# igd-geo/schwarzwald

Hardware: AMD Instinct MI355X
Metric: Mpoints/s end-to-end tile (Morton+sort+sample) (higher is better)
Workload: dtype u64 keys / f64 positions

## Files before the change

schwarzwald_amd/csrc/swz_api.hip:

```cpp
#include <algorithm>
#include <cstring>

#include "swz_device.h"
#include "swz_internal.h"

int swz_ctx::get(const char* name, size_t bytes, void** out) {
  swz::DevBuf& b = bufs[name];
  if (bytes == 0) bytes = 16;
  if (b.cap < bytes) {
    const size_t old_cap = b.cap;
    if (b.ptr) {
      SWZ_HIP(this, hipStreamSynchronize(stream));
      free_buf(b);
    }
    size_t want = bytes + bytes / 16;
    const size_t minimal = (want + 255) & ~size_t(255);
    if (old_cap) {
      if (strncmp(name, "tl_", 3) == 0 || strncmp(name, "tiler_store", 11) == 0) want = std::max(want, 2 * old_cap);
      else want = std::max(want, std::min(2 * old_cap, bytes + (size_t(1) << 30)));
    }
    want = (want + 255) & ~size_t(255);
    hipError_t e = hipMalloc(&b.ptr, want);
    if (const char* fa = opt("SWZ_FAIL_ALLOC")) {
      const size_t fl = strlen(fa);
      const bool hit = fl && fa[fl - 1] == '*' ? strncmp(fa, name, fl - 1) == 0 : strcmp(fa, name) == 0;
      if (e == hipSuccess && hit) {
        (void)hipFree(b.ptr);
        b.ptr = nullptr;
        e = hipErrorOutOfMemory;
      }
    }
    if (e == hipErrorOutOfMemory) {
      (void)hipGetLastError();
      SWZ_HIP(this, hipStreamSynchronize(stream));
      for (auto& kv : bufs) {
        const std::string& nm = kv.first;
        const bool level_scratch = nm.compare(0, 3, "md_") == 0 || nm.compare(0, 3, "sp_") == 0 || nm.compare(0, 3, "pm_") == 0;
        const bool shared_root = md_shard_root_published && nm.size() >= 3 && nm.compare(nm.size() - 3, 3, "_sr") == 0;
        const bool tiler_scratch = tiler_scratch_dead && nm.compare(0, 3, "tl_") == 0;
        if ((level_scratch || tiler_scratch) && !shared_root && kv.second.ptr && kv.second.epoch < scratch_epoch && &kv.second != &b)
          free_buf(kv.second);
      }
      e = hipMalloc(&b.ptr, want);
      if (e == hipErrorOutOfMemory && want > minimal) {
        (void)hipGetLastError();
        want = minimal;
        e = hipMalloc(&b.ptr, want);
      }
    }
    if (e != hipSuccess) {
      b.ptr = nullptr;
      std::vector<std::pair<size_t, std::string>> held;
      size_t total = 0;
      for (const auto& kv : bufs) {
        if (kv.second.host) continue;
        total += kv.second.cap;
        if (kv.second.cap) held.emplace_back(kv.second.cap, kv.first);
      }
      std::sort(held.rbegin(), held.rend());
      size_t free_b = 0, total_b = 0;
      (void)hipMemGetInfo(&free_b, &total_b);
      std::string top;
      for (size_t i = 0; i < held.size() && i < 14; ++i)
        top += " " + held[i].second + "=" + std::to_string(held[i].first >> 20) + "M";
      return fail(SWZ_ERR_HIP, std::string("hipMalloc(") + name + ", " + std::to_string(want) + " bytes): " + hipGetErrorString(e) +
                                 "; workspace holds " + std::to_string(total >> 20) + " MiB, device free " +
                                 std::to_string(free_b >> 20) + " of " + std::to_string(total_b >> 20) + " MiB; largest:" + top);
    }
    b.cap = want;
    if (const char* e = opt("SWZ_POISON")) {
      const char* only = opt("SWZ_POISON_ONLY");
      if (!only || strstr(name, only)) SWZ_HIP(this, hipMemsetAsync(b.ptr, atoi(e), want, stream));
    }
  }
  b.epoch = scratch_epoch;
  *out = b.ptr;
  return SWZ_OK;
}

void swz_ctx::release_all() {
  if (stream) (void)hipStreamSynchronize(stream);
  for (auto& kv : bufs) free_buf(kv.second);
  bufs.clear();
}

void swz_ctx::free_buf(swz::DevBuf& b) {
  if (b.ptr && b.ptr == sbi_clean_ptr) sbi_clean_ptr = nullptr;
  if (b.ptr && b.ptr == mq_qpos_buf) mq_qpos_buf = nullptr;
  if (b.ptr) (void)(b.host ? hipHostFree(b.ptr) : hipFree(b.ptr));
  b.ptr = nullptr;
  b.cap = 0;
  b.host = false;
}

uint64_t swz_ctx::held_bytes() const {
  uint64_t s = 0;
  for (const auto& kv : bufs)
    if (!kv.second.host) s += kv.second.cap;
  return s;
}

uint64_t swz_ctx::held_host_bytes() const {
  uint64_t s = 0;
  for (const auto& kv : bufs)
    if (kv.second.host) s += kv.second.cap;
  return s;
}

hipEvent_t swz_ctx::take_event() {
  if (!event_pool.empty()) {
    hipEvent_t e = event_pool.back();
    event_pool.pop_back();
    return e;
  }
  hipEvent_t e = nullptr;
  (void)hipEventCreate(&e);
  return e;
}

void swz_ctx::prof_begin(const char*) {
  if (!profile) return;
  cur_e0_ = take_event();
  (void)hipEventRecord(cur_e0_, stream);
}

void swz_ctx::prof_end(const char* name, uint64_t launches, uint64_t bytes) {
  if (!profile || !cur_e0_) return;
  hipEvent_t e1 = take_event();
  (void)hipEventRecord(e1, stream);
  pending.push_back({name, cur_e0_, e1, launches, bytes});
  cur_e0_ = nullptr;
}

void swz_ctx::prof_collect() {
  for (auto& p : pending) {
    float ms = 0.f;
    if (hipEventSynchronize(p.e1) == hipSuccess && hipEventElapsedTime(&ms, p.e0, p.e1) == hipSuccess) {
      swz::KernelStat& k = kstats[p.name];
      k.launches += p.launches;
      k.total_ms += ms;
      k.bytes += p.bytes;
    }
    event_pool.push_back(p.e0);
    event_pool.push_back(p.e1);
  }
  pending.clear();
}

int swz::read_u32(swz_ctx* c, const uint32_t* d, uint32_t* h) {
  SWZ_HIP(c, hipMemcpyAsync(h, d, 4, hipMemcpyDeviceToHost, c->stream));
  SWZ_HIP(c, hipStreamSynchronize(c->stream));
  return SWZ_OK;
}

int swz::check_params(swz_ctx* c, const swz_tile_params* p) {
  if (!p) return c->fail(SWZ_ERR_BAD_ARG, "params must not be NULL");
  if (p->sampler < SWZ_RANDOM_GRID || p->sampler > SWZ_MIN_DISTANCE_FAST) return c->fail(SWZ_ERR_BAD_ARG, "unknown sampler");
  if (p->sampler == SWZ_MIN_DISTANCE_FAST && (p->flags & SWZ_FLAG_MIN_DISTANCE_PROPERTY))
    return c->fail(SWZ_ERR_BAD_ARG, "SWZ_FLAG_MIN_DISTANCE_PROPERTY with MIN_DISTANCE_FAST: the property mode's order is not defined for "
                                    "a sampler that offers only every n-th point of a node");
  if (p->strategy != SWZ_ACCURATE && p->strategy != SWZ_FAST) return c->fail(SWZ_ERR_BAD_ARG, "unknown strategy");
  if (!(p->spacing_at_root > 0.f)) return c->fail(SWZ_ERR_BAD_ARG, "spacing_at_root must be > 0");
  if (p->strategy == SWZ_FAST && p->fast_concurrency == 0)
    return c->fail(SWZ_ERR_BAD_ARG, "FAST needs fast_concurrency >= 1");
  return SWZ_OK;
}

const char* swz::sharded_sampler_refusal(int sampler) {
  if (sampler != SWZ_MIN_DISTANCE_FAST) return nullptr;
  return "MIN_DISTANCE_FAST cannot be sharded: the root offers every fourth point of ITS Morton-ordered range, counted across the "
         "shards' octants, and a shard does not know how many points the lower shards hold in front of its own";
}

static std::string g_create_error;

namespace {

int upload(swz_ctx* c, void* dst, const void* src, size_t bytes) {
  if (bytes == 0) return SWZ_OK;
  SWZ_HIP(c, hipMemcpyAsync(dst, src, bytes, hipMemcpyHostToDevice, c->stream));
  return SWZ_OK;
}
int download(swz_ctx* c, void* dst, const void* src, size_t bytes) {
  if (bytes == 0) return SWZ_OK;
  SWZ_HIP(c, hipMemcpyAsync(dst, src, bytes, hipMemcpyDeviceToHost, c->stream));
  return SWZ_OK;
}
int sync(swz_ctx* c) {
  SWZ_HIP(c, hipStreamSynchronize(c->stream));
  c->prof_collect();
  return SWZ_OK;
}
int check_n(swz_ctx* c, uint64_t n) {
  if (n > 0xFFFF0000ull) return c->fail(SWZ_ERR_TOO_MANY_POINTS, "more than 2^32-65536 points in one batch");
  return SWZ_OK;
}
int check_bounds(swz_ctx* c, const double mn[3], const double mx[3]) {
  if (!mn || !mx) return c->fail(SWZ_ERR_BAD_ARG, "bounds must not be NULL");
  for (int a = 0; a < 3; ++a)
    if (!(mx[a] > mn[a])) return c->fail(SWZ_ERR_BAD_ARG, "bounds must have positive extent on every axis");
  return SWZ_OK;
}

}

extern "C" {

int swz_abi_version(void) { return SWZ_ABI_VERSION; }

int swz_create(swz_ctx** ctx_out, int device) {
  if (!ctx_out) return SWZ_ERR_BAD_ARG;
  *ctx_out = nullptr;
  int count = 0;
  hipError_t e = hipGetDeviceCount(&count);
  if (e != hipSuccess || count <= 0) {
    g_create_error = std::string("swz_create: no usable HIP device (") +
                     (e != hipSuccess ? hipGetErrorString(e) : "device count is 0") +
                     "); this library has no CPU fallback";
    return SWZ_ERR_HIP;
  }
  if (device < 0 || device >= count) {
    g_create_error = "swz_create: device ordinal out of range";
    return SWZ_ERR_BAD_ARG;
  }
  e = hipSetDevice(device);
  if (e != hipSuccess) {
    g_create_error = std::string("swz_create: hipSetDevice: ") + hipGetErrorString(e);
    return SWZ_ERR_HIP;
  }
  swz_ctx* c = new swz_ctx();
  c->device = device;
  e = hipStreamCreateWithFlags(&c->own_stream, hipStreamNonBlocking);
  if (e != hipSuccess) {
    g_create_error = std::string("swz_create: hipStreamCreate: ") + hipGetErrorString(e);
    delete c;
    return SWZ_ERR_HIP;
  }
  c->stream = c->own_stream;
  extern char** environ;
  for (char** e = environ; e && *e; ++e) {
    if (std::strncmp(*e, "SWZ_", 4) != 0) continue;
    const char* eq = std::strchr(*e, '=');
    if (eq) c->options[std::string(*e, (size_t)(eq - *e))] = std::string(eq + 1);
  }
  *ctx_out = c;
  return SWZ_OK;
}

int swz_set_option(swz_ctx* c, const char* name, const char* value) {
  if (!c || !name) return SWZ_ERR_BAD_ARG;
  if (value) c->options[name] = value; else c->options.erase(name);
  return SWZ_OK;
}

int swz_destroy(swz_ctx* c) {
  if (!c) return SWZ_OK;
  (void)hipSetDevice(c->device);
  if (c->nodes_tiler) {
    (void)swz_tiler_destroy(c->nodes_tiler);
    c->nodes_tiler = nullptr;
  }
  swz::shard_free(c);
  c->release_all();
  c->prof_collect();
  for (hipEvent_t e : c->event_pool) (void)hipEventDestroy(e);
  for (hipStream_t st : c->aux_streams) (void)hipStreamDestroy(st);
  if (c->own_stream) (void)hipStreamDestroy(c->own_stream);
  delete c;
  return SWZ_OK;
}

const char* swz_last_error(const swz_ctx* c) { return c ? c->err.c_str() : g_create_error.c_str(); }

int swz_set_stream(swz_ctx* c, void* hip_stream) {
  if (!c) return SWZ_ERR_BAD_ARG;
  SWZ_HIP(c, hipStreamSynchronize(c->stream));
  c->stream = hip_stream == SWZ_OWN_STREAM ? c->own_stream : reinterpret_cast<hipStream_t>(hip_stream);
  return SWZ_OK;
}

int swz_release_workspace(swz_ctx* c) {
  if (!c) return SWZ_ERR_BAD_ARG;
  SWZ_HIP(c, hipSetDevice(c->device));
  if (c->tiler_active) return c->fail(SWZ_ERR_BAD_ARG, "swz_release_workspace: a tiler of this context keeps its node store in the workspace");
  swz::shard_free(c);
  c->release_all();
  return SWZ_OK;
}

uint64_t swz_workspace_bytes(const swz_ctx* c) { return c ? c->held_bytes() : 0; }

int swz_host_alloc_pinned(uint64_t bytes, void** out) {
  if (!out) return SWZ_ERR_BAD_ARG;
  *out = nullptr;
  return hipHostMalloc(out, bytes ? bytes : 1, hipHostMallocDefault) == hipSuccess ? SWZ_OK : SWZ_ERR_HIP;
}
int swz_host_free_pinned(void* p) { return (!p || hipHostFree(p) == hipSuccess) ? SWZ_OK : SWZ_ERR_HIP; }

int swz_device_alloc(uint64_t bytes, void** d_out) {
  if (!d_out) return SWZ_ERR_BAD_ARG;
  *d_out = nullptr;
  return hipMalloc(d_out, bytes ? bytes : 1) == hipSuccess ? SWZ_OK : SWZ_ERR_HIP;
}
int swz_device_alloc_on(swz_ctx* c, uint64_t bytes, void** d_out) {
  if (!c || !d_out) return SWZ_ERR_BAD_ARG;
  *d_out = nullptr;
  SWZ_HIP(c, hipSetDevice(c->device));
  SWZ_HIP(c, hipMalloc(d_out, bytes ? bytes : 1));
  return SWZ_OK;
}
int swz_device_free(void* d_ptr) { return (!d_ptr || hipFree(d_ptr) == hipSuccess) ? SWZ_OK : SWZ_ERR_HIP; }
static bool is_mapped_host_memory(const void* p) {
  hipPointerAttribute_t at{};
  if (hipPointerGetAttributes(&at, p) != hipSuccess) {
    (void)hipGetLastError();
    return false;
  }
  return at.type == hipMemoryTypeHost;
}
int swz_copy_to_host(swz_ctx* c, void* dst_host, const void* d_src, uint64_t bytes) {
  if (!c) return SWZ_ERR_BAD_ARG;
  SWZ_HIP(c, hipSetDevice(c->device));
  if (bytes && is_mapped_host_memory(d_src)) {
    SWZ_HIP(c, hipStreamSynchronize(c->stream));
    std::memcpy(dst_host, d_src, bytes);
    return SWZ_OK;
  }
  if (bytes) SWZ_HIP(c, hipMemcpyAsync(dst_host, d_src, bytes, hipMemcpyDeviceToHost, c->stream));
  SWZ_HIP(c, hipStreamSynchronize(c->stream));
  return SWZ_OK;
}
int swz_copy_to_device(swz_ctx* c, void* d_dst, const void* src_host, uint64_t bytes) {
  if (!c) return SWZ_ERR_BAD_ARG;
  SWZ_HIP(c, hipSetDevice(c->device));
  if (bytes && is_mapped_host_memory(d_dst)) {
    SWZ_HIP(c, hipStreamSynchronize(c->stream));
    std::memcpy(d_dst, src_host, bytes);
    return SWZ_OK;
  }
  if (bytes) SWZ_HIP(c, hipMemcpyAsync(d_dst, src_host, bytes, hipMemcpyHostToDevice, c->stream));
  SWZ_HIP(c, hipStreamSynchronize(c->stream));
  return SWZ_OK;
}

int swz_profile_enable(swz_ctx* c, int enabled) {
  if (!c) return SWZ_ERR_BAD_ARG;
  c->profile = enabled != 0;
  return SWZ_OK;
}
int swz_profile_reset(swz_ctx* c) {
  if (!c) return SWZ_ERR_BAD_ARG;
  SWZ_TRY(sync(c));
  c->kstats.clear();
  return SWZ_OK;
}
int swz_profile_get(swz_ctx* c, swz_kernel_stat* out, uint32_t max_stats, uint32_t* num_out) {
  if (!c || !num_out) return SWZ_ERR_BAD_ARG;
  SWZ_TRY(sync(c));
  uint32_t k = 0;
  for (const auto& kv : c->kstats) {
    if (k < max_stats && out) {
      std::memset(&out[k], 0, sizeof(out[k]));
      std::strncpy(out[k].name, kv.first.c_str(), sizeof(out[k].name) - 1);
      out[k].launches = kv.second.launches;
      out[k].total_ms = kv.second.total_ms;
      out[k].algorithmic_bytes = kv.second.bytes;
    }
    ++k;
  }
  *num_out = k;
  return SWZ_OK;
}

int swz_morton_encode_device(swz_ctx* c, double* d_xyz, uint64_t n, const double bmin[3], const double bmax[3],
                             uint64_t* d_keys_out) {
  if (!c) return SWZ_ERR_BAD_ARG;
  SWZ_HIP(c, hipSetDevice(c->device));
  SWZ_TRY(check_n(c, n));
  SWZ_TRY(check_bounds(c, bmin, bmax));
  if (n && (!d_xyz || !d_keys_out)) return c->fail(SWZ_ERR_BAD_ARG, "swz_morton_encode_device: NULL buffer");
  SWZ_TRY(swz::encode_device(c, d_xyz, (uint32_t)n, bmin, bmax, d_keys_out));
  return sync(c);
}

int swz_morton_encode(swz_ctx* c, double* xyz, uint64_t n, const double bmin[3], const double bmax[3],
                      uint64_t* keys_out) {
  if (!c) return SWZ_ERR_BAD_ARG;
  SWZ_HIP(c, hipSetDevice(c->device));
  SWZ_TRY(check_n(c, n));
  SWZ_TRY(check_bounds(c, bmin, bmax));
  if (n == 0) return SWZ_OK;
  if (!xyz || !keys_out) return c->fail(SWZ_ERR_BAD_ARG, "swz_morton_encode: NULL buffer");
  double* d_xyz = nullptr;
  uint64_t* d_keys = nullptr;
  SWZ_TRY(c->get("h_xyz", (size_t)n * 3, &d_xyz));
  SWZ_TRY(c->get("h_keys", (size_t)n, &d_keys));
  SWZ_TRY(upload(c, d_xyz, xyz, (size_t)n * 24));
  SWZ_TRY(swz::encode_device(c, d_xyz, (uint32_t)n, bmin, bmax, d_keys));
  SWZ_TRY(download(c, keys_out, d_keys, (size_t)n * 8));
  SWZ_TRY(download(c, xyz, d_xyz, (size_t)n * 24));
  return sync(c);
}

int swz_sort_by_key_device(swz_ctx* c, const uint64_t* d_keys, uint64_t n, uint32_t* d_perm_out,
                           uint64_t* d_keys_sorted_out) {
  if (!c) return SWZ_ERR_BAD_ARG;
  SWZ_HIP(c, hipSetDevice(c->device));
  SWZ_TRY(check_n(c, n));
  if (n == 0) return SWZ_OK;
  if (!d_keys || !d_perm_out) return c->fail(SWZ_ERR_BAD_ARG, "swz_sort_by_key_device: NULL buffer");
  uint64_t *kin = nullptr, *kout = d_keys_sorted_out;
  uint32_t* vtmp = nullptr;
  SWZ_TRY(c->get("sort_keys_b", (size_t)n, &kin));
  SWZ_TRY(c->get("sort_vals_b", (size_t)n, &vtmp));
  if (!kout) SWZ_TRY(c->get("sort_keys_a", (size_t)n, &kout));
  SWZ_HIP(c, hipMemcpyAsync(kin, d_keys, (size_t)n * 8, hipMemcpyDeviceToDevice, c->stream));
  SWZ_TRY(swz::radix_sort_pairs(c, kin, vtmp, kout, d_perm_out, (uint32_t)n, true));
  return sync(c);
}

int swz_sort_by_key(swz_ctx* c, const uint64_t* keys, uint64_t n, uint32_t* perm_out, uint64_t* keys_sorted_out) {
  if (!c) return SWZ_ERR_BAD_ARG;
  SWZ_HIP(c, hipSetDevice(c->device));
  SWZ_TRY(check_n(c, n));
  if (n == 0) return SWZ_OK;
  if (!keys || !perm_out) return c->fail(SWZ_ERR_BAD_ARG, "swz_sort_by_key: NULL buffer");
  uint64_t *ka = nullptr, *kb = nullptr;
  uint32_t *va = nullptr, *vb = nullptr;
  SWZ_TRY(c->get("sort_keys_a", (size_t)n, &ka));
  SWZ_TRY(c->get("sort_keys_b", (size_t)n, &kb));
  SWZ_TRY(c->get("sort_vals_a", (size_t)n, &va));
  SWZ_TRY(c->get("sort_vals_b", (size_t)n, &vb));
  SWZ_TRY(upload(c, kb, keys, (size_t)n * 8));
  SWZ_TRY(swz::radix_sort_pairs(c, kb, vb, ka, va, (uint32_t)n, true));
  SWZ_TRY(download(c, perm_out, va, (size_t)n * 4));
  if (keys_sorted_out) SWZ_TRY(download(c, keys_sorted_out, ka, (size_t)n * 8));
  return sync(c);
}

int swz_generate_uniform_device(swz_ctx* c, uint64_t seed, uint64_t first_point, uint64_t n, double* d_xyz_out) {
  if (!c) return SWZ_ERR_BAD_ARG;
  SWZ_HIP(c, hipSetDevice(c->device));
  if (n && !d_xyz_out) return c->fail(SWZ_ERR_BAD_ARG, "swz_generate_uniform_device: NULL buffer");
  SWZ_TRY(swz::generate_uniform_device(c, seed, first_point, n, d_xyz_out));
  return sync(c);
}

int swz_tile_device(swz_ctx* c, double* d_xyz, uint64_t n, const double bmin[3], const double bmax[3],
                    const swz_tile_params* params, uint64_t* d_keys_out, uint32_t* d_perm_out, int8_t* d_level_out,
                    uint32_t* d_dup_mask_out, swz_tile_stats* stats) {
  if (!c) return SWZ_ERR_BAD_ARG;
  SWZ_HIP(c, hipSetDevice(c->device));
  if (c->opt("SWZ_SYNC_ENTRY")) SWZ_HIP(c, hipDeviceSynchronize());
  SWZ_TRY(check_n(c, n));
  SWZ_TRY(check_bounds(c, bmin, bmax));
  SWZ_TRY(swz::check_params(c, params));
  if (stats) std::memset(stats, 0, sizeof(*stats));
  if (stats) {
    stats->max_level = -1;
    stats->fast_start_levels = -1;
  }
  if (n == 0) return SWZ_OK;
  if (!d_xyz || !d_keys_out || !d_perm_out || !d_level_out)
    return c->fail(SWZ_ERR_BAD_ARG, "swz_tile_device: NULL buffer");
  swz::TileDeviceOut out{d_keys_out, d_perm_out, d_level_out, d_dup_mask_out};
  int st = swz::tile_device(c, d_xyz, (uint32_t)n, bmin, bmax, *params, out, stats);
  int st2 = sync(c);
  return st != SWZ_OK ? st : st2;
}

int swz_tile(swz_ctx* c, double* xyz, uint64_t n, const double bmin[3], const double bmax[3],
             const swz_tile_params* params, uint64_t* keys_out, uint32_t* perm_out, int8_t* level_out,
             uint32_t* dup_mask_out, swz_tile_stats* stats) {
  if (!c) return SWZ_ERR_BAD_ARG;
  SWZ_HIP(c, hipSetDevice(c->device));
  SWZ_TRY(check_n(c, n));
  SWZ_TRY(check_bounds(c, bmin, bmax));
  SWZ_TRY(swz::check_params(c, params));
  if (stats) {
    std::memset(stats, 0, sizeof(*stats));
    stats->max_level = -1;
    stats->fast_start_levels = -1;
  }
  if (n == 0) return SWZ_OK;
  if (!xyz || !keys_out || !perm_out || !level_out) return c->fail(SWZ_ERR_BAD_ARG, "swz_tile: NULL buffer");
  double* d_xyz = nullptr;
  uint64_t* d_keys = nullptr;
  uint32_t *d_perm = nullptr, *d_dup = nullptr;
  int8_t* d_level = nullptr;
  SWZ_TRY(c->get("h_xyz", (size_t)n * 3, &d_xyz));
  SWZ_TRY(c->get("h_keys", (size_t)n, &d_keys));
  SWZ_TRY(c->get("h_perm", (size_t)n, &d_perm));
  SWZ_TRY(c->get("h_level", (size_t)n, &d_level));
  if (dup_mask_out) SWZ_TRY(c->get("h_dup", (size_t)n, &d_dup));
  SWZ_TRY(upload(c, d_xyz, xyz, (size_t)n * 24));
  swz::TileDeviceOut out{d_keys, d_perm, d_level, d_dup};
  int st = swz::tile_device(c, d_xyz, (uint32_t)n, bmin, bmax, *params, out, stats);
  if (st != SWZ_OK) {
    (void)sync(c);
    return st;
  }
  SWZ_TRY(download(c, keys_out, d_keys, (size_t)n * 8));
  SWZ_TRY(download(c, perm_out, d_perm, (size_t)n * 4));
  SWZ_TRY(download(c, level_out, d_level, (size_t)n));
  if (dup_mask_out) SWZ_TRY(download(c, dup_mask_out, d_dup, (size_t)n * 4));
  SWZ_TRY(download(c, xyz, d_xyz, (size_t)n * 24));
  return sync(c);
}

int swz_partition_by_octant_device(swz_ctx* c, const uint64_t* d_keys, uint64_t n, uint32_t* d_perm_out,
                                   uint64_t counts_out[8]) {
  if (!c || !counts_out) return SWZ_ERR_BAD_ARG;
  SWZ_HIP(c, hipSetDevice(c->device));
  SWZ_TRY(check_n(c, n));
  for (int o = 0; o < 8; ++o) counts_out[o] = 0;
  if (n == 0) return SWZ_OK;
  if (!d_keys || !d_perm_out) return c->fail(SWZ_ERR_BAD_ARG, "swz_partition_by_octant_device: NULL buffer");
  SWZ_TRY(swz::partition_top_digit(c, d_keys, (uint32_t)n, d_perm_out, counts_out));
  return sync(c);
}

int swz_shard_presort_device(swz_ctx* c, const double* d_xyz_local, uint64_t n, const double bmin[3],
                             const double bmax[3], const swz_tile_params* params, uint64_t ghost_capacity) {
  if (!c) return SWZ_ERR_BAD_ARG;
  SWZ_HIP(c, hipSetDevice(c->device));
  SWZ_TRY(check_n(c, n + ghost_capacity));
  SWZ_TRY(check_bounds(c, bmin, bmax));
  SWZ_TRY(swz::check_params(c, params));
  if (const char* why = swz::sharded_sampler_refusal(params->sampler)) return c->fail(SWZ_ERR_BAD_ARG, why);
  if (n && !d_xyz_local) return c->fail(SWZ_ERR_BAD_ARG, "swz_shard_presort_device: NULL buffer");
  if (n == 0) return SWZ_OK;
  int st = swz::shard_presort_device(c, d_xyz_local, (uint32_t)n, bmin, bmax, *params, (uint32_t)ghost_capacity);
  int st2 = sync(c);
  return st != SWZ_OK ? st : st2;
}

int swz_shard_begin_device(swz_ctx* c, const double* d_xyz_local, uint64_t n, const double bmin[3],
                           const double bmax[3], const swz_tile_params* params, const swz_shard_info* shard,
                           uint64_t* num_root_taken_out) {
  if (!c) return SWZ_ERR_BAD_ARG;
  SWZ_HIP(c, hipSetDevice(c->device));
  if (!shard) return c->fail(SWZ_ERR_BAD_ARG, "shard info must not be NULL");
  SWZ_TRY(check_n(c, n + shard->num_ghosts));
  SWZ_TRY(check_bounds(c, bmin, bmax));
  SWZ_TRY(swz::check_params(c, params));
  if (const char* why = swz::sharded_sampler_refusal(params->sampler)) return c->fail(SWZ_ERR_BAD_ARG, why);
  if ((n && !d_xyz_local) || (shard->num_ghosts && !shard->d_ghost_xyz))
    return c->fail(SWZ_ERR_BAD_ARG, "swz_shard_begin_device: NULL buffer");
  if (num_root_taken_out) *num_root_taken_out = 0;
  if (n == 0) {
    return swz::shard_begin_empty(c);
  }
  int st = swz::shard_begin_device(c, d_xyz_local, (uint32_t)n, bmin, bmax, *params, shard->global_points,
                                   shard->d_ghost_xyz, (uint32_t)shard->num_ghosts, num_root_taken_out);
  int st2 = sync(c);
  return st != SWZ_OK ? st : st2;
}

int swz_shard_root_taken_device(swz_ctx* c, double* d_xyz_out) {
  if (!c) return SWZ_ERR_BAD_ARG;
  SWZ_HIP(c, hipSetDevice(c->device));
  SWZ_TRY(swz::shard_root_taken_device(c, d_xyz_out));
  return sync(c);
}

int swz_shard_finish_device(swz_ctx* c, uint64_t* d_keys_out, uint32_t* d_perm_out, int8_t* d_level_out,
                            swz_tile_stats* stats) {
  if (!c) return SWZ_ERR_BAD_ARG;
  SWZ_HIP(c, hipSetDevice(c->device));
  if (stats) {
    std::memset(stats, 0, sizeof(*stats));
    stats->max_level = -1;
    stats->fast_start_levels = -1;
  }
  int st = swz::shard_finish_device(c, d_keys_out, d_perm_out, d_level_out, stats);
  int st2 = sync(c);
  return st != SWZ_OK ? st : st2;
}

int swz_shard_fast_begin_device(swz_ctx* c, const double* d_xyz_local, uint64_t n, const double bmin[3], const double bmax[3],
                                const swz_tile_params* params, uint32_t* prefix_counts_out) {
  if (!c) return SWZ_ERR_BAD_ARG;
  SWZ_HIP(c, hipSetDevice(c->device));
  SWZ_TRY(check_n(c, n));
  SWZ_TRY(check_bounds(c, bmin, bmax));
  SWZ_TRY(swz::check_params(c, params));
  if (const char* why = swz::sharded_sampler_refusal(params->sampler)) return c->fail(SWZ_ERR_BAD_ARG, why);
  if ((n && !d_xyz_local) || !prefix_counts_out) return c->fail(SWZ_ERR_BAD_ARG, "swz_shard_fast_begin_device: NULL buffer");
  int st = swz::shard_fast_begin_device(c, d_xyz_local, (uint32_t)n, bmin, bmax, *params, prefix_counts_out);
  int st2 = sync(c);
  return st != SWZ_OK ? st : st2;
}
int swz_shard_fast_run(swz_ctx* c, int32_t start_level, uint64_t* num_root_candidates_out) {
  if (!c || !num_root_candidates_out) return SWZ_ERR_BAD_ARG;
  SWZ_HIP(c, hipSetDevice(c->device));
  int st = swz::shard_fast_run_device(c, start_level, num_root_candidates_out);
  int st2 = sync(c);
  return st != SWZ_OK ? st : st2;
}
int swz_shard_fast_root_candidates_device(swz_ctx* c, uint64_t* d_keys_out, double* d_xyz_out) {
  if (!c) return SWZ_ERR_BAD_ARG;
  SWZ_HIP(c, hipSetDevice(c->device));
  SWZ_TRY(swz::shard_fast_root_candidates_device(c, d_keys_out, d_xyz_out));
  return sync(c);
}
int swz_shard_fast_set_root_device(swz_ctx* c, const uint8_t* d_taken) {
  if (!c) return SWZ_ERR_BAD_ARG;
  SWZ_HIP(c, hipSetDevice(c->device));
  SWZ_TRY(swz::shard_fast_set_root_device(c, d_taken));
  return sync(c);
}
int swz_shard_fast_finish_device(swz_ctx* c, uint64_t* d_keys_out, uint32_t* d_perm_out, int8_t* d_level_out, uint32_t* d_dup_out,
                                 swz_tile_stats* stats) {
  if (!c) return SWZ_ERR_BAD_ARG;
  SWZ_HIP(c, hipSetDevice(c->device));
  if (stats) {
    std::memset(stats, 0, sizeof(*stats));
    stats->max_level = -1;
    stats->fast_start_levels = -1;
  }
  int st = swz::shard_fast_finish_device(c, d_keys_out, d_perm_out, d_level_out, d_dup_out, stats);
  int st2 = sync(c);
  return st != SWZ_OK ? st : st2;
}

int swz_sample_points(swz_ctx* c, int sampler, uint64_t max_points_per_node, const uint64_t* keys,
                      const uint32_t* idx, uint64_t n, const double* xyz, uint64_t num_points, uint64_t node_key,
                      int32_t node_level, const double root_min[3], const double root_max[3], float spacing_at_root,
                      int behaviour, uint8_t* taken_out, uint64_t* num_taken_out) {
  if (!c) return SWZ_ERR_BAD_ARG;
  SWZ_HIP(c, hipSetDevice(c->device));
  SWZ_TRY(check_n(c, n));
  SWZ_TRY(check_n(c, num_points));
  SWZ_TRY(check_bounds(c, root_min, root_max));
  if (sampler < SWZ_RANDOM_GRID || sampler > SWZ_MIN_DISTANCE_FAST) return c->fail(SWZ_ERR_BAD_ARG, "unknown sampler");
  if (node_level < -1 || node_level > 20) return c->fail(SWZ_ERR_BAD_ARG, "node_level out of range");
  if (num_taken_out) *num_taken_out = 0;
  if (n == 0) return SWZ_OK;
  if (!keys || !idx || !xyz || !taken_out) return c->fail(SWZ_ERR_BAD_ARG, "swz_sample_points: NULL buffer");
  double* d_xyz = nullptr;
  uint64_t* d_keys = nullptr;
  uint32_t* d_idx = nullptr;
  uint8_t* d_taken = nullptr;
  SWZ_TRY(c->get("h_xyz", (size_t)num_points * 3, &d_xyz));
  SWZ_TRY(c->get("h_keys", (size_t)n, &d_keys));
  SWZ_TRY(c->get("h_perm", (size_t)n, &d_idx));
  SWZ_TRY(c->get("h_taken", (size_t)n, &d_taken));
  SWZ_TRY(upload(c, d_xyz, xyz, (size_t)num_points * 24));
  SWZ_TRY(upload(c, d_keys, keys, (size_t)n * 8));
  SWZ_TRY(upload(c, d_idx, idx, (size_t)n * 4));
  int st = swz::sample_points_device(c, sampler, max_points_per_node, d_keys, d_idx, (uint32_t)n, d_xyz, node_key,
                                     node_level, root_min, root_max, spacing_at_root, behaviour, d_taken,
                                     num_taken_out);
  if (st != SWZ_OK) {
    (void)sync(c);
    return st;
  }
  SWZ_TRY(download(c, taken_out, d_taken, (size_t)n));
  return sync(c);
}

int swz_sample_points_device(swz_ctx* c, int sampler, uint64_t max_points_per_node, const uint64_t* d_keys, const uint32_t* d_idx,
                             uint64_t n, const double* d_xyz, uint64_t num_points, uint64_t node_key, int32_t node_level,
                             const double root_min[3], const double root_max[3], float spacing_at_root, int behaviour,
                             uint8_t* d_taken_out, uint64_t* num_taken_out) {
  if (!c) return SWZ_ERR_BAD_ARG;
  SWZ_HIP(c, hipSetDevice(c->device));
  SWZ_TRY(check_n(c, n));
  SWZ_TRY(check_n(c, num_points));
  SWZ_TRY(check_bounds(c, root_min, root_max));
  if (sampler < SWZ_RANDOM_GRID || sampler > SWZ_MIN_DISTANCE_FAST) return c->fail(SWZ_ERR_BAD_ARG, "unknown sampler");
  if (node_level < -1 || node_level > 20) return c->fail(SWZ_ERR_BAD_ARG, "node_level out of range");
  if (num_taken_out) *num_taken_out = 0;
  if (n == 0) return SWZ_OK;
  if (!d_keys || !d_idx || !d_xyz || !d_taken_out) return c->fail(SWZ_ERR_BAD_ARG, "swz_sample_points_device: NULL buffer");
  int st = swz::sample_points_device(c, sampler, max_points_per_node, d_keys, d_idx, (uint32_t)n, d_xyz, node_key, node_level, root_min,
                                     root_max, spacing_at_root, behaviour, d_taken_out, num_taken_out);
  int st2 = sync(c);
  return st != SWZ_OK ? st : st2;
}

int swz_build_node_lists(swz_ctx* c, const uint64_t* keys_sorted, const int8_t* level, uint64_t n,
                         uint32_t* order_out, uint64_t max_nodes, int8_t* node_level_out, uint64_t* node_key_out,
                         uint64_t* node_offset_out, uint64_t* node_count_out, uint64_t* num_nodes_out) {
  if (!c || !num_nodes_out) return SWZ_ERR_BAD_ARG;
  *num_nodes_out = 0;
  if (n == 0) return SWZ_OK;
  if (!keys_sorted || !level || !order_out) return c->fail(SWZ_ERR_BAD_ARG, "swz_build_node_lists: NULL buffer");
  uint64_t hist[23] = {0};
  for (uint64_t i = 0; i < n; ++i) {
    const int l = level[i];
    if (l < -1 || l > 20) return c->fail(SWZ_ERR_BAD_ARG, "level out of range");
    hist[l + 2]++;
  }
  for (int l = 1; l < 23; ++l) hist[l] += hist[l - 1];
  for (uint64_t i = 0; i < n; ++i) order_out[hist[level[i] + 1]++] = (uint32_t)i;
  uint64_t nn = 0;
  uint64_t i = 0;
  while (i < n) {
    const uint64_t p = order_out[i];
    const int l = level[p];
    const uint32_t sh = (l < 0) ? 63u : swz::level_shift(l);
    const uint64_t prefix = keys_sorted[p] >> sh;
    uint64_t j = i + 1;
    while (j < n && level[order_out[j]] == l && (keys_sorted[order_out[j]] >> sh) == prefix) ++j;
    if (nn < max_nodes && node_level_out && node_key_out && node_offset_out && node_count_out) {
      node_level_out[nn] = (int8_t)l;
      node_key_out[nn] = (l < 0) ? 0 : (prefix << sh);
      node_offset_out[nn] = i;
      node_count_out[nn] = j - i;
    }
    ++nn;
    i = j;
  }
  *num_nodes_out = nn;
  if (nn > max_nodes) return c->fail(SWZ_ERR_BAD_ARG, "max_nodes too small");
  return SWZ_OK;
}

}
```

schwarzwald_amd/csrc/swz_internal.h:

```cpp
#pragma once

#include <hip/hip_runtime.h>
#include <stdint.h>

#include <map>
#include <cstdio>
#include <cstdlib>
#include <string>
#include <vector>

#include "../../include/swz_gpu.h"

namespace swz {

constexpr uint32_t MAX_LEVELS = 21;

struct DevBuf {
  void* ptr = nullptr;
  size_t cap = 0;
  uint64_t epoch = 0;
  bool host = false;
};

struct KernelStat {
  uint64_t launches = 0;
  double total_ms = 0.0;
  uint64_t bytes = 0;
};

struct PendingEvent {
  std::string name;
  hipEvent_t e0, e1;
  uint64_t launches;
  uint64_t bytes;
};

}

struct swz_ctx {
  int device = 0;
  hipStream_t own_stream = nullptr;
  hipStream_t stream = nullptr;
  std::string err;
  std::map<std::string, swz::DevBuf> bufs;
  bool profile = false;
  std::map<std::string, swz::KernelStat> kstats;
  std::vector<swz::PendingEvent> pending;
  std::vector<hipEvent_t> event_pool;
  std::vector<hipStream_t> aux_streams;

  int fail(int code, const std::string& msg) {
    err = msg;
    return code;
  }
  int hip_fail(hipError_t e, const char* what, const char* file, int line) {
    err = std::string(what) + ": " + hipGetErrorString(e) + " (" + file + ":" + std::to_string(line) + ")";
    return SWZ_ERR_HIP;
  }

  uint64_t scratch_epoch = 1;
  void next_scratch_epoch() { ++scratch_epoch; }
  int get(const char* name, size_t bytes, void** out);
  template <typename T>
  int get(const char* name, size_t count, T** out) {
    return get(name, count * sizeof(T), reinterpret_cast<void**>(out));
  }
  void release_all();
  void free_buf(swz::DevBuf& b);
  uint64_t held_bytes() const;
  uint64_t held_host_bytes() const;

  hipEvent_t take_event();
  void prof_begin(const char* name);
  void prof_end(const char* name, uint64_t launches, uint64_t bytes);
  void prof_collect();
  hipEvent_t cur_e0_ = nullptr;
  void* shard = nullptr;
  const void* md_shard_root = nullptr;
  bool md_shard_root_published = false;
  const void* sbi_clean_ptr = nullptr;
  size_t sbi_clean_bytes = 0;
  const void* mq_qpos_buf = nullptr;
  const void* mq_qpos_keys = nullptr;
  uint32_t mq_qpos_m = 0;
  bool tiler_active = false;
  swz_tiler* nodes_tiler = nullptr;
  bool tiler_scratch_dead = false;
  std::map<std::string, std::string> options;
  const char* opt(const char* name) const {
    const auto it = options.find(name);
    return it == options.end() ? nullptr : it->second.c_str();
  }
  long opt_int(const char* name, long def) const {
    const char* v = opt(name);
    return v ? (long)atoll(v) : def;
  }
  double opt_num(const char* name, double def) const {
    const char* v = opt(name);
    return v ? atof(v) : def;
  }
  bool opt_on(const char* name, bool def) const {
    const char* v = opt(name);
    return v ? atoi(v) != 0 : def;
  }
};

#define SWZ_HIP(ctx, expr)                                                \
  do {                                                                    \
    hipError_t _e = (expr);                                               \
    if (_e != hipSuccess) return (ctx)->hip_fail(_e, #expr, __FILE__, __LINE__); \
  } while (0)

#define SWZ_TRY(expr)            \
  do {                           \
    int _s = (expr);             \
    if (_s != SWZ_OK) return _s; \
  } while (0)

#define SWZ_LAUNCH_CHECK(ctx) SWZ_HIP(ctx, hipGetLastError())

namespace swz {

inline uint32_t div_up(uint64_t a, uint64_t b) { return (uint32_t)((a + b - 1) / b); }

struct ProfScope {
  swz_ctx* c;
  const char* name;
  uint64_t launches, bytes;
  ProfScope(swz_ctx* ctx, const char* n, uint64_t b, uint64_t l = 1) : c(ctx), name(n), launches(l), bytes(b) {
    c->prof_begin(name);
  }
  ~ProfScope() { c->prof_end(name, launches, bytes); }
};

#define SWZ_STAGE(ctx, what)                                                              \
  do {                                                                                    \
    if ((ctx)->opt("SWZ_TRACE")) {                                                            \
      const hipError_t _e = hipStreamSynchronize((ctx)->stream);                          \
      fprintf(stderr, "[swz trace] %s:%d %s -> %s\n", __FILE__, __LINE__, what, hipGetErrorString(_e)); \
      fflush(stderr);                                                                     \
    }                                                                                     \
  } while (0)

inline hipError_t memset_large(void* p, int value, size_t bytes, hipStream_t stream) {
  const size_t piece = size_t(1) << 30;
  for (size_t at = 0; at < bytes; at += piece) {
    const hipError_t e = hipMemsetAsync(static_cast<char*>(p) + at, value, bytes - at < piece ? bytes - at : piece, stream);
    if (e != hipSuccess) return e;
  }
  return hipSuccess;
}

int read_u32(swz_ctx* c, const uint32_t* d, uint32_t* h);

int encode_device(swz_ctx* c, double* d_xyz, uint32_t n, const double bmin[3], const double bmax[3],
                  uint64_t* d_keys);
int generate_uniform_device(swz_ctx* c, uint64_t seed, uint64_t first, uint64_t n, double* d_xyz);
int check_params(swz_ctx* c, const swz_tile_params* p);
const char* sharded_sampler_refusal(int sampler);

int radix_sort_pairs(swz_ctx* c, uint64_t* d_keys_in, uint32_t* d_vals_tmp, uint64_t* d_keys_out,
                     uint32_t* d_vals_out, uint32_t n, bool vals_identity);

int scan_exclusive_u32(swz_ctx* c, const uint32_t* d_in, uint32_t* d_out, uint64_t n, uint32_t* d_total,
                       const char* tag);

int gather_positions(swz_ctx* c, const double* d_xyz, const uint32_t* d_perm, uint32_t n, double* d_x,
                     double* d_y, double* d_z);

struct TileDeviceOut {
  uint64_t* keys;
  uint32_t* perm;
  int8_t* level;
  uint32_t* dup;
};

int tile_device(swz_ctx* c, double* d_xyz, uint32_t n, const double bmin[3], const double bmax[3],
                const swz_tile_params& p, const TileDeviceOut& out, swz_tile_stats* stats);

int shard_begin_device(swz_ctx* c, const double* d_xyz_local, uint32_t n, const double bmin[3],
                       const double bmax[3], const swz_tile_params& p, uint64_t global_points,
                       const double* d_ghost_xyz, uint32_t ghosts, uint64_t* num_root_taken);
int shard_presort_device(swz_ctx* c, const double* d_xyz_local, uint32_t n, const double bmin[3], const double bmax[3],
                         const swz_tile_params& p, uint32_t ghost_capacity);
int shard_root_taken_device(swz_ctx* c, double* d_xyz_out);
int shard_finish_device(swz_ctx* c, uint64_t* d_keys_out, uint32_t* d_perm_out, int8_t* d_level_out,
                        swz_tile_stats* stats);
int shard_begin_empty(swz_ctx* c);
void shard_free(swz_ctx* c);
int shard_fast_begin_device(swz_ctx* c, const double* d_xyz_local, uint32_t n, const double bmin[3], const double bmax[3],
                            const swz_tile_params& p, uint32_t* counts_host);
int shard_fast_run_device(swz_ctx* c, int start_level, uint64_t* num_root_candidates);
int shard_fast_root_candidates_device(swz_ctx* c, uint64_t* d_keys_out, double* d_xyz_out);
int shard_fast_set_root_device(swz_ctx* c, const uint8_t* d_taken);
int shard_fast_finish_device(swz_ctx* c, uint64_t* d_keys_out, uint32_t* d_perm_out, int8_t* d_level_out, uint32_t* d_dup_out,
                             swz_tile_stats* stats);
int partition_top_digit(swz_ctx* c, const uint64_t* d_keys, uint32_t n, uint32_t* d_perm_out, uint64_t octants[8]);
int partition_by_top_byte(swz_ctx* c, const uint64_t* d_keys, uint32_t n, uint32_t* d_perm_out, uint32_t starts[256]);

int sample_points_device(swz_ctx* c, int sampler, uint64_t max_points, const uint64_t* d_keys,
                         const uint32_t* d_idx, uint32_t n, const double* d_xyz, uint64_t node_key,
                         int32_t node_level, const double rmin[3], const double rmax[3], float spacing,
                         int behaviour, uint8_t* d_taken, uint64_t* num_taken);

}
```

schwarzwald_amd/csrc/swz_md.h:

```cpp
#pragma once
#include "swz_level.h"

namespace swz {

struct MdPeerView {
  const uint4* rec = nullptr;
  const uint64_t* qpos = nullptr;
  const uint8_t* state = nullptr;
  const float4* ovf = nullptr;
  const uint32_t* gridmap = nullptr;
  const uint32_t* round_word = nullptr;
  const uint32_t* perm = nullptr;
  const double* xyz = nullptr;
  const uint32_t* aidx = nullptr;
  uint32_t ncells = 0, rg = 0, cell_shift = 0;
  uint32_t npoints = 0;
  int status = 0;
  int entered = 0;
};
struct MdShardRoot {
  int shard = 0, shards = 1;
  MdPeerView* views = nullptr;
  void (*barrier)(void*) = nullptr;
  void* barrier_arg = nullptr;
};

struct KeyMetric {
  bool ok = false;
  double T = 0.0;
  float f_lo = 0.f;
  float f_hi = 0.f;
};
KeyMetric key_metric(const swz_ctx* c, const LevelPlan& plan, const SortedPoints& sp);
int key_point_ids(swz_ctx* c, const ActiveSet& as, const SortedPoints& sp, const uint32_t** ids);
bool min_distance_level_uses_keys(const swz_ctx* c, const LevelPlan& plan, const SortedPoints& sp);
bool level_decides_on_keys(const swz_ctx* c, const LevelPlan& plan, const SortedPoints& sp);
struct MdLevel {
  const LevelPlan& plan;
  const ActiveSet& as;
  const SortedPoints& sp;
  const LevelBuffers& lb;
  uint32_t num_nodes, sample_nodes, sample_points;
  bool all_sampled;
  const uint32_t* snode_of = nullptr;
  KeyMetric km;
  uint32_t occupied[12] = {0};
  bool sampled_hist = false;
  double pop[4] = {0, 0, 0, 0};
  bool have_pop = false;
};
int md_clamp_cell_levels(uint32_t sample_nodes, int cl);
int md_count_cells_exact(swz_ctx* c, const MdLevel& L, uint32_t occupied[12]);
int md_active_positions(swz_ctx* c, const MdLevel& L, size_t per_point, const double** X, const double** Y, const double** Z);

int min_distance_keys_level(swz_ctx* c, const MdLevel& L, int cl, uint32_t* rounds_out, bool* used,
                            const MdShardRoot* shard_root = nullptr, bool* direct = nullptr);
int min_distance_block_level(swz_ctx* c, const MdLevel& L, bool* done);
int min_distance_sparse_level(swz_ctx* c, const MdLevel& L, int cl, uint32_t* rounds_out, bool* used);
int min_distance_rounds_level(swz_ctx* c, const MdLevel& L, uint32_t* rounds_out, bool* used);
int min_distance_sweep_level(swz_ctx* c, const MdLevel& L, int cl, uint32_t* rounds_out);
int min_distance_phases_level(swz_ctx* c, const MdLevel& L, int cl, uint32_t* phases_out);

}
```

schwarzwald_amd/csrc/swz_md.hip:

```cpp
#include <algorithm>
#include <cmath>

#include "swz_md.h"
#include "swz_scan.h"

namespace swz {

__global__ __launch_bounds__(256) void md_node_flag_kernel(const uint8_t* __restrict__ nmode, uint32_t nnodes,
                                                           uint32_t* __restrict__ out) {
  const uint32_t j = blockIdx.x * 256 + threadIdx.x;
  if (j < nnodes) out[j] = nmode[j] == MODE_SAMPLE ? 1u : 0u;
}

__global__ __launch_bounds__(256) void md_cell_hist_kernel(const uint64_t* __restrict__ akey, const uint32_t* __restrict__ nid,
                                                           const uint8_t* __restrict__ nmode, uint32_t m, uint32_t node_shift,
                                                           uint32_t cl_geo, uint32_t skip, uint32_t* __restrict__ hist) {
  __shared__ uint32_t lh[16];
  if (threadIdx.x < 16) lh[threadIdx.x] = 0;
  __syncthreads();
  uint32_t mine = 0;
  for (uint64_t i0 = (uint64_t)blockIdx.x * skip * 256u; i0 < m; i0 += (uint64_t)gridDim.x * skip * 256u) {
    const uint32_t i = (uint32_t)i0 + threadIdx.x;
    uint32_t bin = 0xFFu;
    if (i0 + threadIdx.x < m && nmode[nid[i]] == MODE_SAMPLE) {
      if (i == 0 || nid[i - 1] != nid[i]) {
        bin = 0;
      } else if (cl_geo) {
        const uint64_t diff = ((akey[i] ^ akey[i - 1]) >> (node_shift - 3u * cl_geo)) & ((1ull << (3u * cl_geo)) - 1ull);
        if (diff) bin = cl_geo - (uint32_t)(63 - __clzll((unsigned long long)diff)) / 3u;
      }
    }
    for (uint32_t b = 0; b <= cl_geo; ++b) {
      const uint32_t cnt = (uint32_t)__popcll(__ballot(bin == b));
      if (lane_id() == b) mine += cnt;
    }
  }
  if (lane_id() <= cl_geo && mine) atomicAdd(&lh[lane_id()], mine);
  __syncthreads();
  if (threadIdx.x < 16 && lh[threadIdx.x]) atomicAdd(&hist[threadIdx.x], lh[threadIdx.x]);
}

constexpr uint32_t MD_POP_SAMPLES = 1u << 16;
__global__ __launch_bounds__(256) void md_cell_pop_kernel(const uint64_t* __restrict__ akey, const uint32_t* __restrict__ nid,
                                                          const uint8_t* __restrict__ nmode, uint32_t m, uint32_t node_shift,
                                                          uint32_t cl_geo, unsigned long long* __restrict__ out) {
  const uint32_t t = blockIdx.x * 256 + threadIdx.x;
  if (t >= MD_POP_SAMPLES) return;
  const uint32_t i = (uint32_t)(((uint64_t)t * m) / MD_POP_SAMPLES);
  if (i >= m || nmode[nid[i]] != MODE_SAMPLE) return;
  const uint64_t key = akey[i];
  for (uint32_t k = 0; k <= 3u && k <= cl_geo; ++k) {
    const uint32_t sh = node_shift - 3u * (cl_geo - k);
    const uint64_t pre = key >> sh;
    uint32_t lo = 0, hi = i;
    while (lo < hi) {
      const uint32_t mid = lo + (hi - lo) / 2u;
      if ((akey[mid] >> sh) < pre) lo = mid + 1u; else hi = mid;
    }
    const uint32_t first = lo;
    lo = i;
    hi = m;
    while (lo < hi) {
      const uint32_t mid = lo + (hi - lo) / 2u;
      if ((akey[mid] >> sh) <= pre) lo = mid + 1u; else hi = mid;
    }
    atomicAdd(&out[k], (unsigned long long)(lo - first));
  }
  atomicAdd(&out[4], 1ull);
}

__global__ __launch_bounds__(256) void md_gather_active_kernel(const uint32_t* __restrict__ aidx, uint32_t m,
                                                               const double* __restrict__ X,
                                                               const double* __restrict__ Y,
                                                               const double* __restrict__ Z, double* __restrict__ ax,
                                                               double* __restrict__ ay, double* __restrict__ az) {
  const uint32_t i = blockIdx.x * 256 + threadIdx.x;
  if (i >= m) return;
  const uint32_t s = aidx[i];
  ax[i] = X[s];
  ay[i] = Y[s];
  az[i] = Z[s];
}

__global__ __launch_bounds__(256) void pm_clear_taken_kernel(const uint32_t* __restrict__ nid, const uint8_t* __restrict__ nmode,
                                                             uint32_t m, uint8_t* __restrict__ taken) {
  const uint32_t i = blockIdx.x * 256 + threadIdx.x;
  if (i < m && nmode[nid[i]] == MODE_SAMPLE) taken[i] = 0;
}

int md_clamp_cell_levels(uint32_t sample_nodes, int cl) {
  while (cl > 0 && (double)sample_nodes * std::pow(8.0, cl) > 2147483648.0) --cl;
  return cl;
}

static int count_cells(swz_ctx* c, const MdLevel& L, uint32_t skip, uint32_t occupied[12]) {
  const uint32_t m = L.as.m;
  uint32_t* d_hist = nullptr;
  SWZ_TRY(c->get("md_hist", (size_t)16, &d_hist));
  SWZ_HIP(c, hipMemsetAsync(d_hist, 0, 64, c->stream));
  const uint32_t tiles = div_up(m, 256);
  const uint32_t sampled_tiles = div_up(tiles, skip);
  hipLaunchKernelGGL(md_cell_hist_kernel, dim3(std::min<uint32_t>(sampled_tiles, 4096u)), dim3(256), 0, c->stream, L.as.akey,
                     L.lb.nid, L.lb.nmode, m, L.plan.node_shift, (uint32_t)L.plan.cell_levels_geo, skip, d_hist);
  SWZ_LAUNCH_CHECK(c);
  SWZ_STAGE(c, "md cell hist");
  uint32_t h[16];
  SWZ_HIP(c, hipMemcpyAsync(h, d_hist, 64, hipMemcpyDeviceToHost, c->stream));
  SWZ_HIP(c, hipStreamSynchronize(c->stream));
  const double scale = skip == 1 ? 1.0 : (double)m / (double)std::min<uint64_t>(m, (uint64_t)sampled_tiles * 256u);
  double run = 0;
  for (int b = 0; b < 12; ++b) {
    run += h[b];
    occupied[b] = (uint32_t)std::min<double>(run * scale, (double)m);
  }
  return SWZ_OK;
}
int md_count_cells_exact(swz_ctx* c, const MdLevel& L, uint32_t occupied[12]) { return count_cells(c, L, 1u, occupied); }

static int md_populations(swz_ctx* c, MdLevel& L) {
  if (L.have_pop) return SWZ_OK;
  unsigned long long* d_pop = nullptr;
  SWZ_TRY(c->get("md_pop", (size_t)8, &d_pop));
  SWZ_HIP(c, hipMemsetAsync(d_pop, 0, 64, c->stream));
  hipLaunchKernelGGL(md_cell_pop_kernel, dim3(MD_POP_SAMPLES / 256), dim3(256), 0, c->stream, L.as.akey, L.lb.nid, L.lb.nmode, L.as.m,
                     L.plan.node_shift, (uint32_t)L.plan.cell_levels_geo, d_pop);
  SWZ_LAUNCH_CHECK(c);
  SWZ_STAGE(c, "md cell pop");
  unsigned long long h[5];
  SWZ_HIP(c, hipMemcpyAsync(h, d_pop, 40, hipMemcpyDeviceToHost, c->stream));
  SWZ_HIP(c, hipStreamSynchronize(c->stream));
  for (int k = 0; k < 4; ++k) L.pop[k] = h[4] ? (double)h[k] / (double)h[4] : 1e30;
  L.have_pop = true;
  return SWZ_OK;
}

static int survey(swz_ctx* c, MdLevel& L) {
  const uint32_t skip = std::max(1u, L.as.m >> 23);
  L.sampled_hist = skip > 1u;
  SWZ_TRY(count_cells(c, L, skip, L.occupied));
  if (!L.plan.md_property) SWZ_TRY(md_populations(c, L));
  uint32_t* snode = nullptr;
  SWZ_TRY(c->get("md_snode", (size_t)L.num_nodes, &snode));
  hipLaunchKernelGGL(md_node_flag_kernel, dim3(div_up(L.num_nodes, 256)), dim3(256), 0, c->stream, L.lb.nmode, L.num_nodes, snode);
  SWZ_LAUNCH_CHECK(c);
  SWZ_TRY(scan_exclusive_u32(c, snode, snode, L.num_nodes, nullptr, "mdn"));
  L.snode_of = snode;
  L.km = key_metric(c, L.plan, L.sp);
  return SWZ_OK;
}

int md_active_positions(swz_ctx* c, const MdLevel& L, size_t per_point, const double** X, const double** Y, const double** Z) {
  *X = L.sp.X;
  *Y = L.sp.Y;
  *Z = L.sp.Z;
  if (!L.as.aidx) return SWZ_OK;
  const uint32_t m = L.as.m;
  double* ax = nullptr;
  SWZ_TRY(c->get("md_pos", (size_t)m * per_point, &ax));
  hipLaunchKernelGGL(md_gather_active_kernel, dim3(div_up(m, 256)), dim3(256), 0, c->stream, L.as.aidx, m, L.sp.X, L.sp.Y, L.sp.Z, ax,
                     ax + m, ax + 2 * (size_t)m);
  SWZ_LAUNCH_CHECK(c);
  *X = ax;
  *Y = ax + m;
  *Z = ax + 2 * (size_t)m;
  return SWZ_OK;
}

static int sweep_cell_levels(const swz_ctx* c, const MdLevel& L) {
  const LevelPlan& plan = L.plan;
  int cl = plan.cell_levels_geo;
  const double avg = (double)L.sample_points / (double)L.sample_nodes;
  const double per_cell = 8.0;
  const double max_pop = 160.0;
  while (cl > 0 && plan.cell_levels_geo - cl < 3 && (double)L.sample_points / (double)std::max(1u, L.occupied[cl]) < per_cell &&
         L.pop[plan.cell_levels_geo - cl + 1] <= max_pop)
    --cl;
  cl = md_clamp_cell_levels(L.sample_nodes, cl);
  if (const long coarsen = c->opt_int("SWZ_MD_COARSEN", 0))
    if (avg / std::pow(8.0, cl) >= c->opt_num("SWZ_MD_COARSEN_MIN", 32.0)) cl = std::max(0, cl - (int)coarsen);
  return cl;
}

static int phases_cell_levels(swz_ctx* c, MdLevel& L, int* cl_out) {
  const LevelPlan& plan = L.plan;
  const double node_ext = (plan.root.maxx - plan.root.minx) / std::pow(2.0, plan.level + 1);
  const double r0 = node_ext / std::pow(2.0, plan.cell_levels_geo) / plan.spacing_node;
  int cl = plan.cell_levels_geo;
  if (cl > 0 && (double)L.sample_points / (double)std::max(1u, L.occupied[cl]) < 24.0 && 0.75 * 8.0 * r0 * r0 * r0 <= 48.0) {
    SWZ_TRY(md_populations(c, L));
    if (L.pop[1] <= 1024.0) --cl;
  }
  *cl_out = md_clamp_cell_levels(L.sample_nodes, cl);
  return SWZ_OK;
}

int min_distance_level(swz_ctx* c, const LevelPlan& plan, const ActiveSet& as, const SortedPoints& sp, const LevelBuffers& lb,
                       uint32_t num_nodes, uint32_t sample_nodes, uint32_t sample_points, uint32_t* rounds_out, bool* keys_direct,
                       bool* needs_flush) {
  bool direct = false;
  if (keys_direct) *keys_direct = false;
  if (needs_flush) *needs_flush = false;
  const bool shared = as.gone != nullptr;
  if (shared && !needs_flush) return c->fail(SWZ_ERR_INTERNAL, "MIN_DISTANCE: a level on shared arrays needs a caller that can compact them");
  c->next_scratch_epoch();
  MdLevel L{plan, as, sp, lb, num_nodes, sample_nodes, sample_points, sample_nodes == num_nodes};
  SWZ_TRY(survey(c, L));
  bool used = false;

  if (c->md_shard_root && plan.level == -1) {
    SWZ_TRY(min_distance_keys_level(c, L, plan.cell_levels_geo, rounds_out, &used, static_cast<const MdShardRoot*>(c->md_shard_root)));
    if (!used) return c->fail(SWZ_ERR_INTERNAL, "MIN_DISTANCE root of a sharded batch: the joint sweep needs a level that can be decided on keys");
    return SWZ_OK;
  }

  const int cl_sparse = md_clamp_cell_levels(sample_nodes, plan.cell_levels_geo);
  const bool sparse = (double)sample_points / (double)std::max(1u, L.occupied[cl_sparse]) < c->opt_num("SWZ_MD_SPARSE_LIMIT", 2.0);
  if (sparse && shared) {
    *needs_flush = true;
    return SWZ_OK;
  }
  if (sparse && !(sp.ghosts && plan.level == -1 && !sp.X)) {
    SWZ_TRY(min_distance_block_level(c, L, &used));
    if (used) {
      if (rounds_out) *rounds_out += 1;
      return SWZ_OK;
    }
    SWZ_TRY(min_distance_sparse_level(c, L, cl_sparse, rounds_out, &used));
    if (used) return SWZ_OK;
    if (plan.md_property) {
      hipLaunchKernelGGL(pm_clear_taken_kernel, dim3(div_up(as.m, 256)), dim3(256), 0, c->stream, lb.nid, lb.nmode, as.m, lb.taken);
      SWZ_LAUNCH_CHECK(c);
    }
  }

  if (plan.md_property && L.km.ok) {
    SWZ_TRY(min_distance_rounds_level(c, L, rounds_out, &used));
    if (used) return SWZ_OK;
  }

  int cl = 0;
  if (!plan.md_property || !sp.X) {
    SWZ_TRY(md_populations(c, L));
    cl = sweep_cell_levels(c, L);
    SWZ_TRY(min_distance_keys_level(c, L, cl, rounds_out, &used, nullptr, &direct));
    if (used) {
      if (keys_direct) *keys_direct = direct;
      return SWZ_OK;
    }
  }
  if (shared) {
    *needs_flush = true;
    return SWZ_OK;
  }

  if (!sp.X) return c->fail(SWZ_ERR_INTERNAL, "MIN_DISTANCE: this level needs the positions in Morton order and they were not gathered");
  if (!plan.md_property) return min_distance_sweep_level(c, L, cl, rounds_out);
  SWZ_TRY(phases_cell_levels(c, L, &cl));
  return min_distance_phases_level(c, L, cl, rounds_out);
}

}
```

schwarzwald_amd/csrc/swz_mdkeys.h:

```cpp
#pragma once
#include <string>
#include <vector>

#include "swz_md.h"

namespace swz {

constexpr uint32_t QNONE = 0xFFFFFFFFu;
constexpr unsigned long long QEMPTY = ~0ull;
constexpr uint32_t MQ_WOKEN = 0x80000000u;
constexpr int MQ_LIST_CAP = 128;
constexpr int MQ_FRESH_CAP = 32;
#ifndef MQ_MINW4
#define MQ_MINW4 4
#endif
#ifndef MQ_MINW1
#define MQ_MINW1 6
#endif
constexpr uint32_t MQ_FIRST_ROUND = 2;
constexpr uint32_t MQ_ROUND_DONE = 0xFFFFFFF0u;
constexpr uint32_t MQ_ROUND_FAILED = 0xFFFFFFF1u;

enum : uint8_t { QS_OPEN = 0, QS_TAKEN = 1, QS_DEAD = 2 };

constexpr uint32_t MQ_PEER_SHIFT = 28;
constexpr uint32_t MQ_ID_MASK = (1u << MQ_PEER_SHIFT) - 1u;
struct MqPeers {
  const uint4* rec[8];
  const uint64_t* qpos[8];
  const uint8_t* state[8];
  const float4* ovf[8];
  const uint32_t* gridmap[8];
  const uint32_t* round_word[8];
  const uint32_t* perm[8];
  const double* xyz[8];
  const uint32_t* aidx[8];
  uint32_t shard, shards;
};

struct MqArgs {
  const uint64_t* akey;
  const uint32_t* aidx;
  uint32_t m;
  const uint32_t* nid;
  const uint8_t* nmode;
  const uint32_t* nstart;
  const double* xyz;
  const uint32_t* perm;
  const double* gxyz;
  uint32_t ng;
  uint8_t* taken;
  uint32_t* counters;
  uint64_t* qpos;
  uint8_t* state;
  uint32_t direct;
  uint32_t cpn_shift;
  uint2* cinfo;
  uint32_t* crel;
  uint32_t* csnode;
  uint32_t* gridmap;
  uint32_t* qnbr;
  uint4* rec;
  float4* ovf;
  unsigned long long* slot;
  uint4* qst;
  uint32_t* queue[2];
  uint32_t* qctr;
  uint32_t* qtotal;
  uint32_t* qhead;
  uint32_t nseg, nseg_shift, segcap;
  const uint32_t* snode_of;
  uint32_t cell_shift;
  uint64_t cells_per_node;
  uint32_t cell_bits;
  uint32_t cell_levels;
  uint32_t rg, rg2_shift;
  float f_lo, f_hi;
  double sq_spacing;
  uint32_t patient;
  float lazy_frac;
  uint32_t all_sampled;
  uint32_t group, groups;
  uint32_t no_dead_test;
  uint32_t stats;
  uint32_t chain;
  uint32_t dense_min;
  uint8_t* dirty;
  uint32_t* bulk_round;
  const uint32_t* dlist;
  uint32_t* round_word;
  MqPeers peers;
  const uint8_t* gone;
  uint32_t keep_qpos;
};

constexpr uint32_t MQ_CHAIN = 8;
__host__ __device__ constexpr uint32_t mq_staged(bool peers) { return peers ? 27u : 20u; }
static inline size_t mq_lds_bytes(uint32_t rg, bool peers) {
  return (size_t)(mq_staged(peers) * 2u * rg + MQ_LIST_CAP + MQ_FRESH_CAP) * 16u + MQ_LIST_CAP + MQ_CHAIN * 4u + 128u;
}

struct MqLevel {
  const MdLevel& L;
  int cl;
  const MdShardRoot* shard_root;
  bool* used;
  bool sharded = false;
  std::string sfx;
  MqArgs a{};
  uint64_t grid_entries = 0;
  uint32_t ncells = 0;
  uint32_t occ_cells = 0;
  uint32_t* d_cell_sums = nullptr;
  bool coded = false;
  bool lazy = false, big_cells = false;
  uint32_t groups = 1, ndense = 0;
  std::vector<MqArgs> ga;
  std::vector<hipStream_t> gs;
  uint32_t round = MQ_FIRST_ROUND;
  bool over = false;
};

int mq_count_cells(swz_ctx* c, MqLevel& q);
int mq_alloc_arrays(swz_ctx* c, MqLevel& q);
int mq_build_cell_tables(swz_ctx* c, MqLevel& q);
int mq_list_dense_cells(swz_ctx* c, MqLevel& q);
int mq_start_groups(swz_ctx* c, MqLevel& q);
uint32_t mq_sweep_grid(swz_ctx* c, const MqLevel& q);
void mq_launch_round(const MqLevel& q, uint32_t g, uint32_t sweep_grid);
void mq_set_round_word(hipStream_t stream, uint32_t* word, uint32_t value);
int mq_verify(swz_ctx* c, MqLevel& q);
int mq_commit(swz_ctx* c, MqLevel& q);

}
```

schwarzwald_amd/csrc/swz_mdkeys.hip:

```cpp
#include <algorithm>
#include <chrono>
#include <cmath>
#include <cstdio>
#include <cstdlib>
#include <string>
#include <vector>

#include "swz_mdkeys.h"

namespace swz {

KeyMetric key_metric(const swz_ctx* c, const LevelPlan& plan, const SortedPoints& sp) {
  KeyMetric k;
  if (!sp.xyz || !sp.perm) return k;
  if (!c->opt_on("SWZ_MD_KEYS", true)) return k;
  const double ex = plan.root.maxx - plan.root.minx, ey = plan.root.maxy - plan.root.miny, ez = plan.root.maxz - plan.root.minz;
  if (!(ex > 0.0) || ex != ey || ey != ez) return k;
  const double cell = ex / 2097152.0;
  const double T = std::sqrt(plan.sq_spacing) / cell;
  const double tmin = c->opt_num("SWZ_MD_KEYS_MIN_CELLS", 64.0);
  if (!(T >= tmin) || !(T < 4.0e6)) return k;
  double band = 1.75 + T * 0x1.0p-20;
  band += c->opt_num("SWZ_MD_KEYS_BAND", 0.0);
  const double lo = T - band, hi = T + band;
  float f_lo = 0.f;
  if (lo > 0.0) {
    f_lo = (float)(lo * lo);
    while ((double)f_lo > lo * lo) f_lo = std::nextafterf(f_lo, 0.f);
    f_lo = std::nextafterf(f_lo, 0.f);
  }
  float f_hi = (float)(hi * hi);
  while ((double)f_hi < hi * hi) f_hi = std::nextafterf(f_hi, INFINITY);
  f_hi = std::nextafterf(f_hi, INFINITY);
  k.T = T;
  k.f_lo = f_lo;
  k.f_hi = f_hi;
  k.ok = true;
  return k;
}

__global__ __launch_bounds__(256) void mq_point_ids_kernel(const uint32_t* __restrict__ aidx, const uint32_t* __restrict__ perm, uint32_t m,
                                                           uint32_t ghosts, uint32_t* __restrict__ ids) {
  const uint32_t i = blockIdx.x * 256 + threadIdx.x;
  if (i >= m) return;
  const uint32_t s = aidx ? aidx[i] : i;
  ids[i] = s < ghosts ? perm[s] : ghosts + perm[s];
}
int key_point_ids(swz_ctx* c, const ActiveSet& as, const SortedPoints& sp, const uint32_t** ids) {
  if (!as.aidx && !sp.ghosts) {
    *ids = sp.perm;
    return SWZ_OK;
  }
  uint32_t* d = nullptr;
  SWZ_TRY(c->get("md_qids", (size_t)as.m, &d));
  hipLaunchKernelGGL(mq_point_ids_kernel, dim3(div_up(as.m, 256)), dim3(256), 0, c->stream, as.aidx, sp.perm, as.m, sp.ghosts, d);
  SWZ_LAUNCH_CHECK(c);
  *ids = d;
  return SWZ_OK;
}

bool min_distance_level_uses_keys(const swz_ctx* c, const LevelPlan& plan, const SortedPoints& sp) {
  return key_metric(c, plan, sp).ok;
}

static int mq_fill_args(const swz_ctx* c, MqLevel& q) {
  const MdLevel& L = q.L;
  if (!L.km.ok) {
    q.over = true;
    return SWZ_OK;
  }
  q.sharded = q.shard_root != nullptr && q.shard_root->shards > 1;
  q.sfx = q.sharded ? "_sr" : "";
  MqArgs& a = q.a;
  a.akey = L.as.akey;
  a.aidx = L.as.aidx;
  a.m = L.as.m;
  a.nid = L.lb.nid;
  a.nmode = L.lb.nmode;
  a.nstart = L.lb.nstart;
  a.xyz = L.sp.xyz;
  a.perm = L.sp.perm;
  a.gxyz = L.sp.ghost_xyz;
  a.ng = L.sp.ghosts;
  a.taken = L.lb.taken;
  a.counters = L.lb.counters;
  a.snode_of = L.snode_of;
  a.cells_per_node = 1ull << (3 * q.cl);
  a.cpn_shift = 3u * (uint32_t)q.cl;
  a.cell_levels = (uint32_t)q.cl;
  a.peers.shards = q.sharded ? (uint32_t)q.shard_root->shards : 1u;
  a.peers.shard = q.sharded ? (uint32_t)q.shard_root->shard : 0u;
  a.cell_shift = L.plan.node_shift - 3u * (uint32_t)q.cl;
  a.cell_bits = a.cell_shift / 3u;
  a.f_lo = L.km.f_lo;
  a.f_hi = L.km.f_hi;
  a.sq_spacing = L.plan.sq_spacing;
  a.all_sampled = L.all_sampled ? 1u : 0u;
  a.no_dead_test = c->opt_on("SWZ_MD_NO_DEAD_TEST", false) ? 1u : 0u;
  a.stats = c->opt("SWZ_MD_STATS") ? 1u : 0u;
  a.chain = std::min<uint32_t>(MQ_CHAIN, (uint32_t)std::max(1L, c->opt_int("SWZ_MD_CHAIN", 2)));
  if (a.cell_bits > 21u) q.over = true;
  return SWZ_OK;
}

static int mq_choose_records_and_numbering(const swz_ctx* c, MqLevel& q, bool* direct_out) {
  MqArgs& a = q.a;
  const double r_cell = std::ldexp(1.0, (int)a.cell_bits) / q.L.km.T;
  a.rg = (0.75 * r_cell * r_cell * r_cell <= 12.0) ? 4u : 8u;
  a.rg = c->opt_int("SWZ_MD_KEYS_RG", a.rg) >= 8 ? 8u : 4u;
  a.rg2_shift = a.rg == 4u ? 3u : 4u;
  q.grid_entries = (uint64_t)q.L.sample_nodes * a.cells_per_node;
  const size_t per_cell = sizeof(uint2) + 32u * 4u + 2u * a.rg * sizeof(uint4) + 32u * 8u + sizeof(uint4) + 5u;
  uint64_t max_cells = 0x7FFFFFF0ull;
  if (const char* mc = c->opt("SWZ_MD_DIRECT_MAX_CELLS")) {
    max_cells = std::min<uint64_t>(max_cells, (uint64_t)std::max(0LL, atoll(mc)));
  } else {
    size_t free_b = 0, total_b = 0, held = 0;
    if (hipMemGetInfo(&free_b, &total_b) != hipSuccess) free_b = 0;
    for (const auto& kv : c->bufs)
      if (!kv.second.host && kv.first.compare(0, 4, "md_q") == 0) held += kv.second.cap;
    max_cells = std::min<uint64_t>(max_cells, (uint64_t)((double)(free_b + held) * 0.9 / (double)per_cell));
  }
  const double occupancy = (double)q.L.occupied[q.cl] / (double)std::max<uint64_t>(1, q.grid_entries);
  bool direct = occupancy >= c->opt_num("SWZ_MD_DIRECT_MIN_OCCUPANCY", 0.5);
  if (const char* f = c->opt("SWZ_MD_DIRECT")) direct = atoi(f) != 0;
  a.direct = (direct && !q.sharded && q.grid_entries <= max_cells) ? 1u : 0u;
  if (q.L.as.gone && !a.direct) {
    q.over = true;
    return SWZ_OK;
  }
  if (direct_out) *direct_out = a.direct != 0u;
  *q.used = true;
  return SWZ_OK;
}

struct MqWordGuard {
  swz_ctx* c;
  uint32_t* word = nullptr;
  bool done = false;
  ~MqWordGuard() {
    if (word && !done) {
      mq_set_round_word(c->stream, word, MQ_ROUND_FAILED);
      (void)hipStreamSynchronize(c->stream);
    }
  }
};

static int mq_publish_view(swz_ctx* c, MqLevel& q) {
  MqArgs& a = q.a;
  const ActiveSet& as = q.L.as;
  MdPeerView& mine = q.shard_root->views[q.shard_root->shard];
  int my_status = SWZ_OK;
  if (q.cl < 1 || q.ncells >= (1u << MQ_PEER_SHIFT) || q.L.sample_nodes != 1) my_status = SWZ_ERR_INTERNAL;
  const uint32_t* aidx_sr = nullptr;
  if (as.aidx) {
    uint32_t* cp = nullptr;
    SWZ_TRY(c->get("md_qaidx_sr", (size_t)a.m, &cp));
    SWZ_HIP(c, hipMemcpyAsync(cp, as.aidx, (size_t)a.m * 4, hipMemcpyDeviceToDevice, c->stream));
    aidx_sr = cp;
  }
  SWZ_TRY(c->get("md_qround_sr", (size_t)32, &a.round_word));
  mq_set_round_word(c->stream, a.round_word, MQ_FIRST_ROUND);
  SWZ_LAUNCH_CHECK(c);
  SWZ_HIP(c, hipStreamSynchronize(c->stream));
  mine.rec = a.rec;
  mine.qpos = a.qpos;
  mine.state = a.state;
  mine.ovf = a.ovf;
  mine.gridmap = a.gridmap;
  mine.round_word = a.round_word;
  mine.perm = a.perm;
  mine.xyz = a.xyz;
  mine.aidx = aidx_sr;
  mine.ncells = q.ncells;
  mine.npoints = a.m;
  mine.rg = a.rg;
  mine.cell_shift = a.cell_shift;
  mine.status = my_status;
  mine.entered = 1;
  return SWZ_OK;
}

static int mq_meet_peers(swz_ctx* c, MqLevel& q) {
  MqArgs& a = q.a;
  const MdShardRoot* sr = q.shard_root;
  sr->barrier(sr->barrier_arg);
  for (int p = 0; p < sr->shards; ++p) {
    const MdPeerView& v = sr->views[p];
    if (v.status != SWZ_OK || (v.ncells && (v.rg != a.rg || v.cell_shift != a.cell_shift)))
      return c->fail(SWZ_ERR_INTERNAL, "MIN_DISTANCE root of a sharded batch: shard " + std::to_string(p) +
                                         " cannot take part in the joint sweep (cell levels, cell count or record size differ)");
    if (p < sr->shard && v.ncells) {
      a.peers.rec[p] = v.rec;
      a.peers.qpos[p] = v.qpos;
      a.peers.state[p] = v.state;
      a.peers.ovf[p] = v.ovf;
      a.peers.gridmap[p] = v.gridmap;
      a.peers.round_word[p] = v.round_word;
      a.peers.perm[p] = v.perm;
      a.peers.xyz[p] = v.xyz;
      a.peers.aidx[p] = v.aidx;
    }
  }
  return SWZ_OK;
}

static void mq_schedule(const swz_ctx* c, MqLevel& q) {
  MqArgs& a = q.a;
  const uint32_t sample_nodes = q.L.sample_nodes;
  const double typical_pop = q.L.pop[std::min(3, q.L.plan.cell_levels_geo - q.cl)];
  const bool many_small = q.occ_cells >= (4u << 20) && (double)q.L.sample_points / (double)q.occ_cells <= 128.0;
  a.patient = (uint32_t)c->opt_int("SWZ_MD_PATIENT", many_small ? 1 : 0);
  q.lazy = c->opt_on("SWZ_MD_LAZY", true);
  a.lazy_frac = (float)c->opt_num("SWZ_MD_LAZY_FRAC", many_small ? 0.5 : 0.0);
  q.big_cells = c->opt_on("SWZ_MD_BIG", typical_pop > 256.0);
  uint32_t groups = 1;
  if (sample_nodes >= 2 && !q.big_cells) groups = 2;
  groups = (uint32_t)std::max(1L, std::min(8L, c->opt_int("SWZ_MD_GROUPS", groups)));
  groups = std::min(groups, sample_nodes);
  if (q.sharded) groups = 1;
  q.groups = groups;
}

static int mq_run_rounds(swz_ctx* c, MqLevel& q) {
  const uint32_t groups = q.groups, m = q.a.m;
  const uint32_t sweep_grid = mq_sweep_grid(c, q);
  uint32_t batch = 32, batches_done = 0;
  const bool fixed_batch = c->opt("SWZ_MD_BATCH") != nullptr;
  if (fixed_batch) batch = std::max(1u, (uint32_t)c->opt_int("SWZ_MD_BATCH", 0));
  const auto wall0 = std::chrono::steady_clock::now();
  const double wall_limit = c->opt_num("SWZ_MD_TIME_LIMIT", 900.0);
  uint64_t max_rounds = 8ull * m + 1024;
  if (q.sharded) {
    uint64_t below = 0;
    for (int p = 0; p < q.shard_root->shard; ++p) below += q.shard_root->views[p].npoints;
    max_rounds += 64ull * below + 65536ull;
  }
  max_rounds = (uint64_t)c->opt_int("SWZ_MD_ROUND_LIMIT", (long)max_rounds);
  hipEvent_t fork = nullptr;
  if (groups > 1) {
    fork = c->take_event();
    SWZ_HIP(c, hipEventRecord(fork, c->stream));
    for (uint32_t g = 1; g < groups; ++g) SWZ_HIP(c, hipStreamWaitEvent(q.gs[g], fork, 0));
  }
  std::vector<uint32_t> gleft(groups, 1);
  uint32_t& round = q.round;
  bool running = true;
  while (running) {
    for (uint32_t b = 0; b < batch; ++b, ++round)
      for (uint32_t g = 0; g < groups; ++g) mq_launch_round(q, g, sweep_grid);
    SWZ_LAUNCH_CHECK(c);
    if (!fixed_batch && ++batches_done % 4u == 0u && batch < 128u) batch *= 2u;
    for (uint32_t g = 0; g < groups; ++g)
      SWZ_HIP(c, hipMemcpyAsync(&gleft[g], q.ga[g].qtotal + (round - 1u - MQ_FIRST_ROUND) % 3u, 4, hipMemcpyDeviceToHost, q.gs[g]));
    uint32_t peer_err = 0;
    if (q.sharded) SWZ_HIP(c, hipMemcpyAsync(&peer_err, q.ga[0].counters + CTR_ERROR, 4, hipMemcpyDeviceToHost, q.gs[0]));
    running = false;
    for (uint32_t g = 0; g < groups; ++g) {
      SWZ_HIP(c, hipStreamSynchronize(q.gs[g]));
      running |= gleft[g] != 0u;
    }
    if (peer_err) return c->fail(SWZ_ERR_INTERNAL, "MIN_DISTANCE root of a sharded batch: a lower shard's sweep failed (or a queue overflowed); this shard gives up as well");
    if (std::chrono::duration<double>(std::chrono::steady_clock::now() - wall0).count() > wall_limit) {
      char msg[200];
      snprintf(msg, sizeof(msg), "MIN_DISTANCE sweep on keys exceeded %.0f s: level %d, %u cells, %u rounds", wall_limit, q.L.plan.level,
               q.ncells, round);
      return c->fail(SWZ_ERR_INTERNAL, msg);
    }
    if (round > max_rounds) {
      char msg[160];
      snprintf(msg, sizeof(msg), "MIN_DISTANCE sweep on keys did not terminate: level %d, %u cells, %u rounds", q.L.plan.level, q.ncells, round);
      return c->fail(SWZ_ERR_INTERNAL, msg);
    }
  }
  if (fork) c->event_pool.push_back(fork);
  return SWZ_OK;
}

struct MqTrace {
  bool on = false;
  hipEvent_t ev0 = nullptr, ev1 = nullptr;
};
static void mq_trace_begin(swz_ctx* c, const MqLevel& q, MqTrace& t) {
  t.on = c->opt("SWZ_DEBUG") != nullptr;
  if (!t.on) return;
  const MqArgs& a = q.a;
  const MdLevel& L = q.L;
  fprintf(stderr, "[swz] MIN_DISTANCE level %d on keys: %u pts in %u nodes, %u cells%s (cell levels %d), spacing %.1f key cells, band "
                  "[%.0f, %.0f), records of %u, typical cell %.0f pts, lazy %d (%.2f) patient %u groups %u big %d dense cells %u\n",
          L.plan.level, L.sample_points, L.sample_nodes, q.ncells, a.direct ? " of the grid, numbered directly" : "", q.cl, L.km.T, (double)L.km.f_lo, (double)L.km.f_hi, a.rg - 1u,
          L.pop[std::min(3, L.plan.cell_levels_geo - q.cl)], (int)q.lazy, (double)a.lazy_frac, a.patient, q.groups, (int)q.big_cells, q.ndense);
  t.ev0 = c->take_event();
  t.ev1 = c->take_event();
  (void)hipEventRecord(t.ev0, c->stream);
}
static int mq_trace_end(swz_ctx* c, const MqLevel& q, MqTrace& t) {
  if (!t.on) return SWZ_OK;
  float ms = 0.f;
  (void)hipEventRecord(t.ev1, c->stream);
  (void)hipEventSynchronize(t.ev1);
  (void)hipEventElapsedTime(&ms, t.ev0, t.ev1);
  c->event_pool.push_back(t.ev0);
  c->event_pool.push_back(t.ev1);
  fprintf(stderr, "[swz] MIN_DISTANCE level %d on keys: sweep %.2f ms, %u rounds\n", q.L.plan.level, ms, q.round - MQ_FIRST_ROUND);
  for (uint32_t g = 0; g < q.groups; ++g) {
    uint32_t h[CTR_COUNT];
    SWZ_HIP(c, hipMemcpy(h, q.ga[g].counters, sizeof(h), hipMemcpyDeviceToHost));
    fprintf(stderr, "[swz]   group %u: %u full activations, %u confirms still asleep, %u confirms that lost the claim, %u stalls, %u scans\n", g,
            h[CTR_DBG_HIST], h[CTR_DBG_HIST + 1], h[CTR_DBG_HIST + 2], h[CTR_DBG_HIST + 3], h[CTR_DBG_HIST + 4]);
#ifdef SWZ_MQ_STATS
    {
      const double ns = std::max(1u, h[CTR_DBG_HIST + 15]) * 100.0;
      fprintf(stderr, "[swz]   timed %u full activations (us): first loads %.2f, records + window %.2f, list %.2f, first window (R) %.2f, "
                      "windows + candidates + scans %.2f, publish + wake %.2f, total %.2f\n", h[CTR_DBG_HIST + 15], h[CTR_DBG_HIST + 8] / ns,
              h[CTR_DBG_HIST + 9] / ns, h[CTR_DBG_HIST + 10] / ns, h[CTR_DBG_HIST + 11] / ns, h[CTR_DBG_HIST + 12] / ns, h[CTR_DBG_HIST + 13] / ns,
              h[CTR_DBG_HIST + 14] / ns);
    }
#endif
  }
  return SWZ_OK;
}

#define MQ_STEP(call)            \
  do {                           \
    SWZ_TRY(call);               \
    if (q.over) return SWZ_OK;   \
  } while (0)

int min_distance_keys_level(swz_ctx* c, const MdLevel& L, int cl, uint32_t* rounds_out, bool* used, const MdShardRoot* shard_root,
                            bool* direct_out) {
  *used = false;
  if (direct_out) *direct_out = false;
  MqLevel q{L, cl, shard_root, used};
  MQ_STEP(mq_fill_args(c, q));
  ProfScope ps(c, "sample_min_distance", (uint64_t)L.sample_points * 33ull, 1);
  MQ_STEP(mq_choose_records_and_numbering(c, q, direct_out));
  MQ_STEP(mq_count_cells(c, q));
  SWZ_TRY(mq_alloc_arrays(c, q));
  SWZ_TRY(mq_build_cell_tables(c, q));
  MqWordGuard word_guard{c};
  if (q.sharded) {
    SWZ_TRY(mq_publish_view(c, q));
    word_guard.word = q.a.round_word;
    SWZ_TRY(mq_meet_peers(c, q));
  }
  mq_schedule(c, q);
  SWZ_TRY(mq_list_dense_cells(c, q));
  SWZ_TRY(mq_start_groups(c, q));
  MqTrace trace;
  mq_trace_begin(c, q, trace);
  SWZ_TRY(mq_run_rounds(c, q));
  if (q.sharded) {
    mq_set_round_word(c->stream, q.a.round_word, MQ_ROUND_DONE);
    word_guard.done = true;
    SWZ_LAUNCH_CHECK(c);
  }
  SWZ_TRY(mq_verify(c, q));
  SWZ_TRY(mq_commit(c, q));
  if (rounds_out) *rounds_out += q.round - MQ_FIRST_ROUND;
  return mq_trace_end(c, q, trace);
}

}
```

schwarzwald_amd/csrc/swz_mqbuild.hip:

```cpp
#include <algorithm>
#include <string>
#include <vector>

#include "swz_mdkeys.h"
#include "swz_scan.h"

namespace swz {

__device__ __forceinline__ uint64_t mq_pack(uint64_t key) {
  uint32_t x, y, z;
  key_coords_u32(key, x, y, z);
  return (uint64_t)x | ((uint64_t)y << 21) | ((uint64_t)z << 42);
}
__device__ __forceinline__ bool mq_is_head(const MqArgs& a, uint32_t i) {
  if (!a.all_sampled && a.nmode[a.nid[i]] != MODE_SAMPLE) return false;
  return i == 0 || ((a.akey[i] >> a.cell_shift) != (a.akey[i - 1] >> a.cell_shift));
}

__global__ __launch_bounds__(256) void mq_pack_kernel(const uint64_t* __restrict__ akey, uint32_t m, uint64_t* __restrict__ qpos,
                                                      uint8_t* __restrict__ state) {
  const uint32_t i = blockIdx.x * 256 + threadIdx.x;
  if (i >= m) return;
  qpos[i] = mq_pack(akey[i]);
  state[i] = QS_OPEN;
}

struct MqHeadF {
  MqArgs a;
  __device__ uint32_t operator()(uint32_t i) const { return mq_is_head(a, i) ? 1u : 0u; }
};
struct MqCellBuildG {
  MqArgs a;
  __device__ void operator()(uint32_t i, uint32_t c, uint32_t head) const {
    const uint64_t key = a.akey[i];
    a.qpos[i] = mq_pack(key);
    a.state[i] = QS_OPEN;
    if (!head) return;
    a.cinfo[c].x = i;
    a.crel[c] = (uint32_t)((key >> a.cell_shift) & (a.cells_per_node - 1ull));
    a.csnode[c] = a.all_sampled ? a.nid[i] : a.snode_of[a.nid[i]];
  }
};

__global__ __launch_bounds__(256) void mq_direct_build_kernel(MqArgs a, uint32_t vec) {
  const uint64_t i0 = ((uint64_t)blockIdx.x * 256u + threadIdx.x) * 4u;
  if (i0 >= a.m) return;
  const uint32_t n = a.m - i0 < 4u ? (uint32_t)(a.m - i0) : 4u;
  uint64_t key[6];
  uint64_t q[4];
  if (vec && n == 4u) {
    const ulonglong2 v0 = *reinterpret_cast<const ulonglong2*>(a.akey + i0), v1 = *reinterpret_cast<const ulonglong2*>(a.akey + i0 + 2);
    key[1] = v0.x, key[2] = v0.y, key[3] = v1.x, key[4] = v1.y;
  } else {
#pragma unroll
    for (uint32_t j = 0; j < 4u; ++j) key[1 + j] = j < n ? a.akey[i0 + j] : 0ull;
  }
  key[0] = i0 ? a.akey[i0 - 1u] : 0ull;
  key[5] = i0 + 4u < a.m ? a.akey[i0 + 4u] : 0ull;
  if (!a.keep_qpos) {
#pragma unroll
    for (int j = 0; j < 4; ++j) q[j] = mq_pack(key[1 + j]);
  }
  if (n == 4u) {
    if (!a.keep_qpos) {
      ulonglong2 w0, w1;
      w0.x = q[0], w0.y = q[1], w1.x = q[2], w1.y = q[3];
      *reinterpret_cast<ulonglong2*>(a.qpos + i0) = w0;
      *reinterpret_cast<ulonglong2*>(a.qpos + i0 + 2) = w1;
    }
    uint32_t sw = 0x01010101u * (uint32_t)QS_OPEN;
    if (a.gone) {
      const uint32_t g = *reinterpret_cast<const uint32_t*>(a.gone + i0);
#pragma unroll
      for (int j = 0; j < 4; ++j)
        if ((g >> (8 * j)) & 0xFFu) sw = (sw & ~(0xFFu << (8 * j))) | ((uint32_t)QS_DEAD << (8 * j));
    }
    *reinterpret_cast<uint32_t*>(a.state + i0) = sw;
  } else {
    for (uint32_t j = 0; j < n; ++j) {
      if (!a.keep_qpos) a.qpos[i0 + j] = q[j];
      a.state[i0 + j] = (a.gone && a.gone[i0 + j]) ? (uint8_t)QS_DEAD : (uint8_t)QS_OPEN;
    }
  }
#pragma unroll
  for (uint32_t j = 0; j < 4u; ++j) {
    if (j >= n) break;
    const uint32_t i = (uint32_t)i0 + j;
    const uint64_t pre = key[1 + j] >> a.cell_shift;
    const bool first = i == 0u || (key[j] >> a.cell_shift) != pre;
    const bool last = i + 1u == a.m || (key[2 + j] >> a.cell_shift) != pre;
    if (!first && !last) continue;
    const uint32_t node = a.nid[i];
    if (!a.all_sampled && a.nmode[node] != MODE_SAMPLE) continue;
    const uint64_t g = ((uint64_t)(a.all_sampled ? node : a.snode_of[node]) << a.cpn_shift) | (pre & (a.cells_per_node - 1ull));
    if (first) a.cinfo[g].x = i;
    if (last) a.cinfo[g].y = i + 1u;
  }
}

__global__ __launch_bounds__(256) void mq_cell_end_kernel(MqArgs a, uint32_t ncells) {
  const uint32_t c = blockIdx.x * 256 + threadIdx.x;
  if (c >= ncells) return;
  const uint32_t s = a.cinfo[c].x;
  const uint32_t node_end = a.nstart[a.nid[s] + 1];
  const uint32_t next = (c + 1 < ncells) ? a.cinfo[c + 1].x : a.m;
  const uint32_t e = next < node_end ? next : node_end;
  a.cinfo[c].y = e;
  a.gridmap[(uint64_t)a.csnode[c] * a.cells_per_node + a.crel[c]] = c;
  uint4* r = a.rec + ((size_t)c << a.rg2_shift);
  r[0] = make_uint4(s, 0u, 0u, e);
  r[a.rg] = make_uint4(s, 0u, 1u, e);
  a.qst[c] = make_uint4(QNONE, 0u, 0u, 0u);
}

__device__ __forceinline__ void mq_wave_push(bool want, uint32_t value, uint32_t* qout, uint32_t* cout) {
  const uint64_t m = __ballot(want);
  if (!m) return;
  const int leader = __ffsll((unsigned long long)m) - 1;
  uint32_t base = 0;
  if ((int)lane_id() == leader) base = atomicAdd(cout, (uint32_t)__popcll(m));
  base = __shfl(base, leader, WAVE);
  if (want) qout[base + (uint32_t)__popcll(m & lanemask_lt())] = value;
}

struct MqStart {
  uint32_t* queue[8];
  uint32_t* qctr[8];
  uint32_t groups;
  uint32_t lazy;
};

__global__ __launch_bounds__(256) void mq_nbr_build_kernel(MqArgs a, uint32_t ncells, MqStart st) {
  for (uint64_t cbase = (uint64_t)blockIdx.x * 8u; cbase < ncells; cbase += (uint64_t)gridDim.x * 8u) {
    const uint32_t c = (uint32_t)cbase + threadIdx.x / 32u;
    const uint32_t k = threadIdx.x & 31u;
    const bool in_grid = c < ncells;
    bool in = in_grid;
    if (a.direct && in_grid) {
      const uint2 ci = a.cinfo[c];
      if (k < 2u) a.rec[((size_t)c << a.rg2_shift) + k * a.rg] = make_uint4(ci.x, 0u, k, ci.y);
      in = ci.x != ci.y;
    }
    uint32_t nb = QNONE;
    if (in && k == 13u) {
      nb = c;
    } else if (in && k < 27u) {
      const uint32_t rel = a.direct ? (c & (uint32_t)(a.cells_per_node - 1ull)) : a.crel[c];
      const uint32_t all = (uint32_t)(a.cells_per_node - 1ull);
      const uint32_t mz = all & 0x09249249u, my = mz << 1, mx = mz << 2;
      const uint32_t v[3] = {rel & mx, rel & my, rel & mz};
      const uint32_t mk[3] = {mx, my, mz};
      const uint32_t d[3] = {k / 9u, (k / 3u) % 3u, k % 3u};
      bool inside = true;
      uint32_t nrel = 0;
#pragma unroll
      for (int ax = 0; ax < 3; ++ax) {
        uint32_t w = v[ax];
        if (d[ax] == 0u) {
          inside &= w != 0u;
          w = (w - 1u) & mk[ax];
        } else if (d[ax] == 2u) {
          inside &= w != mk[ax];
          w = ((w | ~mk[ax]) + 1u) & mk[ax];
        }
        nrel |= w;
      }
      if (inside) {
        if (a.peers.shards > 1u) {
          const uint32_t owner = (nrel >> (3u * (a.cell_levels - 1u))) * a.peers.shards / 8u;
          if (owner == a.peers.shard) {
            nb = a.gridmap[nrel];
          } else if (owner < a.peers.shard && a.peers.gridmap[owner]) {
            const uint32_t id = a.peers.gridmap[owner][nrel];
            if (id != QNONE) nb = ((owner + 1u) << MQ_PEER_SHIFT) | id;
          }
        } else if (a.direct) {
          const uint32_t g = (c - rel) | nrel;
          const uint2 cn = a.cinfo[g];
          if (cn.x != cn.y) nb = g;
        } else {
          nb = a.gridmap[(uint64_t)a.csnode[c] * a.cells_per_node + nrel];
        }
      }
    }
    if (in) a.qnbr[(size_t)c * 32 + k] = nb;
    uint32_t best = 0;
    if (st.lazy && in && k < 27u && nb != QNONE && (a.peers.shards <= 1u || (nb >> MQ_PEER_SHIFT) == 0u) && nb < c) best = nb + 1u;
    if (st.lazy) {
#pragma unroll
      for (int off = 16; off >= 1; off >>= 1) best = max(best, (uint32_t)__shfl_xor((int)best, off, 32));
      if (in && best && nb + 1u == best) {
        const uint2 o = a.cinfo[best - 1u];
        const uint32_t bq = o.x + (uint32_t)((float)(o.y - 1u - o.x) * a.lazy_frac);
        a.slot[(size_t)(best - 1u) * 32 + (26u - k)] = (unsigned long long)bq;
        a.qst[c] = make_uint4(a.cinfo[c].x, k, bq, 0u);
      }
    }
    if (a.direct && in_grid && k == 2u && best == 0u) a.qst[c] = make_uint4(QNONE, 0u, 0u, 0u);
    const bool push = in && k == 13u && best == 0u;
    const uint32_t seg = (uint32_t)(cbase >> 3) & (a.nseg - 1u);
    if (st.groups == 1u) {
      mq_wave_push(push, c | MQ_WOKEN, st.queue[0] + (size_t)seg * a.segcap, st.qctr[0] + (size_t)seg * 32u);
    } else {
      const uint32_t g = push ? (a.direct ? c >> a.cpn_shift : a.csnode[c]) % st.groups : 0u;
      for (uint32_t gg = 0; gg < st.groups; ++gg)
        mq_wave_push(push && g == gg, c | MQ_WOKEN, st.queue[gg] + (size_t)seg * a.segcap, st.qctr[gg] + (size_t)seg * 32u);
    }
  }
}

__global__ __launch_bounds__(256) void mq_dense_list_kernel(MqArgs a, uint32_t ncells, uint32_t* __restrict__ list, uint32_t* __restrict__ count) {
  const uint32_t c = blockIdx.x * 256 + threadIdx.x;
  if (c >= ncells) return;
  const uint2 ci = a.cinfo[c];
  if (ci.y - ci.x >= a.dense_min) list[atomicAdd(count, 1u)] = c;
}

int mq_count_cells(swz_ctx* c, MqLevel& q) {
  MqArgs& a = q.a;
  const LevelBuffers& lb = q.L.lb;
  if (a.direct) {
    if (q.L.sample_points == 0) {
      q.over = true;
      return SWZ_OK;
    }
    q.ncells = (uint32_t)q.grid_entries;
  } else {
    SWZ_TRY(fused_scan_sums(c, MqHeadF{a}, a.m, lb.counters + CTR_NUM_CELLS, "mqc", &q.d_cell_sums));
    SWZ_HIP(c, hipMemcpyAsync(&q.ncells, lb.counters + CTR_NUM_CELLS, 4, hipMemcpyDeviceToHost, c->stream));
    SWZ_HIP(c, hipStreamSynchronize(c->stream));
    if (q.ncells == 0 || q.ncells >= 0x7FFFFFFFu) {
      if (q.ncells) *q.used = false;
      q.over = true;
      return SWZ_OK;
    }
  }
  q.occ_cells = a.direct ? std::max(1u, std::min<uint32_t>(q.L.occupied[q.cl], q.ncells)) : q.ncells;
  return SWZ_OK;
}

int mq_alloc_arrays(swz_ctx* c, MqLevel& q) {
  MqArgs& a = q.a;
  const ActiveSet& as = q.L.as;
  const uint32_t m = a.m, ncells = q.ncells;
  const std::string& sfx = q.sfx;
  SWZ_TRY(c->get(("md_qpos" + sfx).c_str(), (size_t)m, &a.qpos));
  SWZ_TRY(c->get(("md_qstate" + sfx).c_str(), (size_t)m, &a.state));
  q.coded = as.gone != nullptr || q.L.plan.take_code != 1;
  if (q.coded) a.taken = a.state;
  a.gone = as.gone;
  a.keep_qpos = (as.gone && c->mq_qpos_buf == a.qpos && c->mq_qpos_keys == as.akey && c->mq_qpos_m == m) ? 1u : 0u;
  c->mq_qpos_buf = q.sharded ? nullptr : a.qpos;
  c->mq_qpos_keys = as.akey;
  c->mq_qpos_m = m;
  SWZ_TRY(c->get(("md_qovf" + sfx).c_str(), (size_t)m, &a.ovf));
  SWZ_TRY(c->get(("md_qcinfo" + sfx).c_str(), (size_t)ncells, &a.cinfo));
  if (!a.direct) {
    uint32_t* cellbuf = nullptr;
    SWZ_TRY(c->get(("md_qcells" + sfx).c_str(), (size_t)ncells * 2, &cellbuf));
    a.crel = cellbuf;
    a.csnode = cellbuf + ncells;
  }
  SWZ_TRY(c->get(("md_qnbr" + sfx).c_str(), (size_t)ncells * 32, &a.qnbr));
  SWZ_TRY(c->get(("md_qrec" + sfx).c_str(), (size_t)ncells * 2 * a.rg, &a.rec));
  SWZ_TRY(c->get(("md_qslot" + sfx).c_str(), (size_t)ncells * 32, &a.slot));
  SWZ_TRY(c->get(("md_qst" + sfx).c_str(), (size_t)ncells, &a.qst));
  SWZ_HIP(c, memset_large(a.slot, 0xFF, (size_t)ncells * 32 * sizeof(unsigned long long), c->stream));
  return SWZ_OK;
}

int mq_build_cell_tables(swz_ctx* c, MqLevel& q) {
  MqArgs& a = q.a;
  const uint32_t m = a.m, ncells = q.ncells;
  if (a.direct) {
    SWZ_HIP(c, memset_large(a.cinfo, 0, (size_t)ncells * sizeof(uint2), c->stream));
    hipLaunchKernelGGL(mq_direct_build_kernel, dim3(div_up(m, 1024)), dim3(256), 0, c->stream, a,
                       ((uintptr_t)a.akey & 15u) == 0 ? 1u : 0u);
    SWZ_LAUNCH_CHECK(c);
  } else {
    SWZ_TRY(c->get(("md_gridmap" + q.sfx).c_str(), (size_t)q.grid_entries, &a.gridmap));
    SWZ_HIP(c, memset_large(a.gridmap, 0xFF, (size_t)q.grid_entries * 4, c->stream));
    SWZ_TRY(fused_scan_apply(c, MqHeadF{a}, MqCellBuildG{a}, m, q.d_cell_sums));
    hipLaunchKernelGGL(mq_cell_end_kernel, dim3(div_up(ncells, 256)), dim3(256), 0, c->stream, a, ncells);
    SWZ_LAUNCH_CHECK(c);
  }
  return SWZ_OK;
}

int mq_list_dense_cells(swz_ctx* c, MqLevel& q) {
  MqArgs& a = q.a;
  const uint32_t m = a.m, ncells = q.ncells;
  q.ndense = 0;
  a.dense_min = 0;
  a.dirty = nullptr;
  if (!(q.big_cells && q.groups == 1 && !q.sharded)) return SWZ_OK;
  const uint32_t dense_min = (uint32_t)std::max(0L, c->opt_int("SWZ_MD_DENSE_MIN", 4096));
  if (!dense_min || m < dense_min) return SWZ_OK;
  uint32_t* dl = nullptr;
  uint32_t* dcount = nullptr;
  SWZ_TRY(c->get("md_qdense", (size_t)(m / dense_min + 1u), &dl));
  SWZ_TRY(c->get("md_qdense_count", (size_t)4, &dcount));
  SWZ_HIP(c, hipMemsetAsync(dcount, 0, 4, c->stream));
  a.dense_min = dense_min;
  hipLaunchKernelGGL(mq_dense_list_kernel, dim3(div_up(ncells, 256)), dim3(256), 0, c->stream, a, ncells, dl, dcount);
  SWZ_LAUNCH_CHECK(c);
  SWZ_HIP(c, hipMemcpyAsync(&q.ndense, dcount, 4, hipMemcpyDeviceToHost, c->stream));
  SWZ_HIP(c, hipStreamSynchronize(c->stream));
  if (q.ndense) {
    SWZ_TRY(c->get("md_qdirty", (size_t)ncells, &a.dirty));
    SWZ_TRY(c->get("md_qbulk", (size_t)ncells, &a.bulk_round));
    SWZ_HIP(c, hipMemsetAsync(a.dirty, 0, (size_t)ncells, c->stream));
    SWZ_HIP(c, hipMemsetAsync(a.bulk_round, 0, (size_t)ncells * 4, c->stream));
    a.dlist = dl;
  } else {
    a.dense_min = 0;
  }
  return SWZ_OK;
}

int mq_start_groups(swz_ctx* c, MqLevel& q) {
  MqArgs& a = q.a;
  const uint32_t groups = q.groups, ncells = q.ncells;
  a.nseg_shift = 5;
  a.nseg = 1u << a.nseg_shift;
  a.segcap = (uint32_t)std::min<uint64_t>(0x7FFFFFF0ull, 2ull * ncells / a.nseg + 4096ull);
  q.ga.assign(groups, a);
  q.gs.assign(groups, c->stream);
  MqStart start{};
  start.groups = groups;
  start.lazy = q.lazy ? 1u : 0u;
  for (uint32_t g = 0; g < groups; ++g) {
    MqArgs& ag = q.ga[g];
    ag.group = g;
    ag.groups = groups;
    const std::string tag = std::to_string(g);
    SWZ_TRY(c->get(("md_qqueue0_g" + tag).c_str(), (size_t)a.nseg * a.segcap, &ag.queue[0]));
    SWZ_TRY(c->get(("md_qqueue1_g" + tag).c_str(), (size_t)a.nseg * a.segcap, &ag.queue[1]));
    SWZ_TRY(c->get(("md_qctr_g" + tag).c_str(), (size_t)6 * a.nseg * 32 + 32, &ag.qctr));
    ag.qhead = ag.qctr + (size_t)3 * a.nseg * 32;
    ag.qtotal = ag.qctr + (size_t)6 * a.nseg * 32;
    SWZ_HIP(c, hipMemsetAsync(ag.qctr, 0, ((size_t)6 * a.nseg * 32 + 32) * sizeof(uint32_t), c->stream));
    if (g > 0) {
      SWZ_TRY(c->get(("md_counters_g" + tag).c_str(), (size_t)CTR_COUNT, &ag.counters));
      SWZ_HIP(c, hipMemsetAsync(ag.counters, 0, CTR_COUNT * sizeof(uint32_t), c->stream));
      while (c->aux_streams.size() < g) {
        hipStream_t stn = nullptr;
        SWZ_HIP(c, hipStreamCreateWithFlags(&stn, hipStreamNonBlocking));
        c->aux_streams.push_back(stn);
      }
      q.gs[g] = c->aux_streams[g - 1];
    }
    start.queue[g] = ag.queue[0];
    start.qctr[g] = ag.qctr;
  }
  hipLaunchKernelGGL(mq_nbr_build_kernel, dim3(std::min<uint32_t>(div_up(ncells, 8), 1u << 20)), dim3(256), 0, c->stream, q.ga[0], ncells, start);
  SWZ_LAUNCH_CHECK(c);
  SWZ_STAGE(c, "mq tables");
  return SWZ_OK;
}

}
```

schwarzwald_amd/csrc/swz_session.hip:

```cpp
#include <algorithm>
#include <string>
#include <vector>

#include "swz_md.h"
#include "swz_session.h"

namespace swz {

static int session_gather_positions(swz_ctx* c, TileSession& t) {
  if (t.sp.X) return SWZ_OK;
  double *X = nullptr, *Y = nullptr, *Z = nullptr;
  SWZ_TRY(c->get("sorted_x", (size_t)t.n + t.front, &X));
  SWZ_TRY(c->get("sorted_y", (size_t)t.n + t.front, &Y));
  SWZ_TRY(c->get("sorted_z", (size_t)t.n + t.front, &Z));
  SWZ_STAGE(c, "sort");
  const uint32_t g = t.sp.ghosts;
  if (g) {
    if (t.next_level <= -1) SWZ_TRY(gather_positions(c, t.sp.ghost_xyz, t.perm, g, X, Y, Z));
    SWZ_TRY(gather_positions(c, t.xyz_in, t.perm + g, t.n - g, X + g, Y + g, Z + g));
  } else {
    X += t.front;
    Y += t.front;
    Z += t.front;
    SWZ_TRY(gather_positions(c, t.xyz_in, t.perm, t.n, X, Y, Z));
  }
  SWZ_STAGE(c, "gather");
  t.sp.X = X;
  t.sp.Y = Y;
  t.sp.Z = Z;
  return SWZ_OK;
}
static int session_need_positions(swz_ctx* c, TileSession& t, const LevelPlan& plan) {
  if (t.sp.X || level_decides_on_keys(c, plan, t.sp)) return SWZ_OK;
  return session_gather_positions(c, t);
}

int session_prepare(swz_ctx* c, TileSession& t, double* d_xyz, uint32_t n, const double bmin[3], const double bmax[3],
                    const swz_tile_params& p, const TileDeviceOut& out, uint32_t front) {
  t = TileSession{};
  t.n = n;
  for (int a = 0; a < 3; ++a) {
    t.bmin[a] = bmin[a];
    t.bmax[a] = bmax[a];
  }
  t.params = p;
  t.keys = out.keys;
  t.perm = out.perm;
  t.level = out.level;
  t.dup = out.dup;
  t.xyz_in = d_xyz;
  uint64_t* keys_b = nullptr;
  uint32_t* vals_b = nullptr;
  SWZ_TRY(c->get("sort_keys_b", (size_t)n, &keys_b));
  SWZ_TRY(c->get("sort_vals_b", (size_t)n, &vals_b));
  SWZ_TRY(encode_device(c, d_xyz, n, bmin, bmax, keys_b));
  SWZ_STAGE(c, "encode");
  SWZ_TRY(radix_sort_pairs(c, keys_b, vals_b, out.keys, out.perm, n, true));
  t.sp = SortedPoints{nullptr, nullptr, nullptr, d_xyz, out.perm};
  t.front = front;
  const LevelPlan top = make_plan(-1, p.sampler, p.max_points_per_node, p.spacing_at_root, p.max_depth, bmin, bmax, false, true);
  SWZ_TRY(session_need_positions(c, t, top));
  if (out.dup) SWZ_HIP(c, hipMemsetAsync(out.dup, 0, (size_t)n * 4, c->stream));
  SWZ_HIP(c, hipMemsetAsync(out.level, 0x80, (size_t)n, c->stream));
  SWZ_TRY(alloc_level_buffers(c, n + front, &t.lb));
  t.key_buf[0] = keys_b;
  t.idx_buf[0] = vals_b;
  t.as = ActiveSet{out.keys, nullptr, n};
  return SWZ_OK;
}

int session_run_levels(swz_ctx* c, TileSession& t, int last_level, int first_mode, bool chains) {
  const uint64_t* pprefix = nullptr;
  uint32_t parents = 0;
  const bool chain_static = chains && first_mode < 0 && t.params.sampler == SWZ_MIN_DISTANCE &&
                            !(t.params.flags & SWZ_FLAG_MIN_DISTANCE_PROPERTY) && !t.sp.ghosts && !t.front && !c->shard &&
                            !c->md_shard_root && c->opt_on("SWZ_MD_DEFER", true);
  LevelChain chain;
  chain.max_gone = c->opt_num("SWZ_MD_DEFER_MAX_GONE", 0.125);
  for (int level = t.next_level; (t.as.gone ? t.as.live : t.as.m) > 0 && level <= last_level; ++level) {
    if (level > 20) return c->fail(SWZ_ERR_INTERNAL, "level loop ran past level 20");
    if (!t.key_buf[t.which]) {
      SWZ_TRY(c->get("active_keys_2", (size_t)t.as.m, &t.key_buf[t.which]));
      SWZ_TRY(c->get("active_idx_2", (size_t)t.as.m, &t.idx_buf[t.which]));
    }
    LevelPlan plan = make_plan(level, t.params.sampler, t.params.max_points_per_node, t.params.spacing_at_root,
                               t.params.max_depth, t.bmin, t.bmax, false, true);
    plan.md_property = (t.params.flags & SWZ_FLAG_MIN_DISTANCE_PROPERTY) != 0;
    chain.may_defer = false;
    if (chain_static && level < 20) {
      const LevelPlan next = make_plan(level + 1, t.params.sampler, t.params.max_points_per_node, t.params.spacing_at_root,
                                       t.params.max_depth, t.bmin, t.bmax, false, true);
      chain.may_defer = !plan.terminal && !plan.reroot && !next.terminal && !next.reroot;
    }
    if (chain.may_defer || t.as.gone) plan.take_code = (uint8_t)(level + 2);
    if (first_mode >= 0 && level == t.next_level) plan.md_property = false;
    if (first_mode >= 0 && level == t.next_level && !plan.terminal) {
      if (first_mode == 1) {
        plan.force_sample = true;
      } else {
        plan.max_points = ~0ull;
      }
    }
    SWZ_TRY(session_need_positions(c, t, plan));
    LevelResult r;
    t.as.parent_prefix = pprefix;
    t.as.parents = pprefix ? parents : 0u;
    SWZ_TRY(level_step(c, plan, t.as, t.sp, t.lb, t.level, t.key_buf[t.which], t.idx_buf[t.which], &r, &chain));
    if (r.needs_flush) {
      if (!t.as.gone) return c->fail(SWZ_ERR_INTERNAL, "a level outside a chain asked for the chain's compaction");
      uint32_t remaining = 0;
      SWZ_TRY(level_flush_chain(c, t.as, t.lb, t.level, t.key_buf[t.which], t.idx_buf[t.which], &remaining));
      t.as = ActiveSet{t.key_buf[t.which], t.idx_buf[t.which], remaining};
      t.which ^= 1;
      --level;
      continue;
    }
    t.visited += t.as.gone ? t.as.live : t.as.m;
    t.nodes += r.num_nodes;
    t.rounds += r.md_rounds;
    t.max_level = level;
    ++t.nlevels;
    if (r.deferred) {
      t.as.gone = t.lb.taken;
      t.as.gone_tiles = r.gone_tiles;
      t.as.live = r.remaining;
    } else {
      t.as = ActiveSet{t.key_buf[t.which], t.idx_buf[t.which], r.remaining};
      t.which ^= 1;
    }
    pprefix = r.node_prefix;
    parents = r.table_nodes;
    t.next_level = level + 1;
  }
  return SWZ_OK;
}

void session_stats(const TileSession& t, swz_tile_stats* stats) {
  if (!stats) return;
  stats->num_nodes = t.nodes;
  stats->points_visited = t.visited;
  stats->max_level = t.max_level;
  stats->fast_start_levels = t.fast_start;
  stats->num_levels = t.nlevels;
  stats->min_distance_rounds = t.rounds;
}

__global__ __launch_bounds__(256) void prefix_bounds_kernel(const uint64_t* __restrict__ keys, uint32_t n,
                                                            uint32_t* __restrict__ starts, uint32_t nbins) {
  const uint32_t b = blockIdx.x * 256 + threadIdx.x;
  if (b > nbins) return;
  if (b == nbins) {
    starts[b] = n;
    return;
  }
  const uint64_t target = (uint64_t)b << 45;
  uint32_t lo = 0, hi = n;
  while (lo < hi) {
    const uint32_t mid = lo + (hi - lo) / 2;
    if (keys[mid] < target) lo = mid + 1; else hi = mid;
  }
  starts[b] = lo;
}

static size_t estimate_start_level_host(const std::vector<uint32_t>& starts6, size_t concurrency) {
  constexpr uint32_t MIN_LEVEL = 3, MAX_LEVEL = 6;
  constexpr float MIN_SCORE = 1.f;
  for (uint32_t level = 0; level < MAX_LEVEL; ++level) {
    const uint32_t digits = level + 1;
    const uint32_t group = 1u << (3 * (6 - digits));
    size_t ranges = 0, large = 0;
    for (uint32_t b = 0; b < (1u << 18); b += group) {
      const uint32_t cnt = starts6[b + group] - starts6[b];
      if (cnt > 0) ++ranges;
      if (cnt >= 100000) ++large;
    }
    float score = 0.f;
    if (!(ranges <= concurrency / 2)) score = static_cast<float>(large) / static_cast<float>(concurrency);
    if (score >= MIN_SCORE) return std::max(level + 1, MIN_LEVEL);
  }
  return MAX_LEVEL;
}

__global__ __launch_bounds__(256) void recon_select_kernel(const int8_t* __restrict__ level,
                                                           const uint32_t* __restrict__ dup, uint32_t n,
                                                           int start_node_level, uint32_t child_bit,
                                                           uint32_t* __restrict__ flags) {
  const uint32_t i = blockIdx.x * 256 + threadIdx.x;
  if (i >= n) return;
  flags[i] = recon_candidate(level, dup, i, start_node_level, child_bit) ? 1u : 0u;
}
__global__ __launch_bounds__(256) void recon_gather_kernel(const uint64_t* __restrict__ keys, uint32_t n,
                                                           const uint32_t* __restrict__ flags_in_scanned,
                                                           const int8_t* __restrict__ level,
                                                           const uint32_t* __restrict__ dup, int start_node_level,
                                                           uint32_t child_bit, uint64_t* __restrict__ okey,
                                                           uint32_t* __restrict__ oidx) {
  const uint32_t i = blockIdx.x * 256 + threadIdx.x;
  if (i >= n) return;
  if (recon_candidate(level, dup, i, start_node_level, child_bit)) {
    const uint32_t o = flags_in_scanned[i];
    okey[o] = keys[i];
    oidx[o] = i;
  }
}
__global__ __launch_bounds__(256) void recon_mark_kernel(const uint32_t* __restrict__ aidx, uint32_t m,
                                                         const uint8_t* __restrict__ taken, uint32_t bit,
                                                         uint32_t* __restrict__ dup) {
  const uint32_t i = blockIdx.x * 256 + threadIdx.x;
  if (i < m && taken[i]) dup[aidx[i]] |= bit;
}

int fast_prefix_counts(swz_ctx* c, const uint64_t* d_keys_sorted, uint32_t n, uint32_t* counts_host) {
  const uint32_t nbins = 1u << 18;
  uint32_t* d_starts = nullptr;
  SWZ_TRY(c->get("fast_starts", (size_t)nbins + 1, &d_starts));
  std::vector<uint32_t> starts(nbins + 1, 0);
  if (n) {
    hipLaunchKernelGGL(prefix_bounds_kernel, dim3(div_up(nbins + 1, 256)), dim3(256), 0, c->stream, d_keys_sorted, n, d_starts, nbins);
    SWZ_LAUNCH_CHECK(c);
    SWZ_HIP(c, hipMemcpyAsync(starts.data(), d_starts, (nbins + 1) * 4, hipMemcpyDeviceToHost, c->stream));
    SWZ_HIP(c, hipStreamSynchronize(c->stream));
  }
  for (uint32_t b = 0; b < nbins; ++b) counts_host[b] = starts[b + 1] - starts[b];
  return SWZ_OK;
}
int fast_start_level_from_counts(const uint64_t* counts, uint32_t concurrency) {
  std::vector<uint32_t> starts((1u << 18) + 1, 0);
  uint64_t run = 0;
  for (uint32_t b = 0; b < (1u << 18); ++b) {
    starts[b] = (uint32_t)std::min<uint64_t>(run, 0xFFFFFFFFull);
    run += counts[b];
  }
  starts[1u << 18] = (uint32_t)std::min<uint64_t>(run, 0xFFFFFFFFull);
  return (int)estimate_start_level_host(starts, concurrency);
}

int fast_start_level(swz_ctx* c, const uint64_t* d_keys_sorted, uint32_t n, uint32_t concurrency, int* start_level) {
  const uint32_t nbins = 1u << 18;
  uint32_t* d_starts = nullptr;
  SWZ_TRY(c->get("fast_starts", (size_t)nbins + 1, &d_starts));
  hipLaunchKernelGGL(prefix_bounds_kernel, dim3(div_up(nbins + 1, 256)), dim3(256), 0, c->stream, d_keys_sorted, n,
                     d_starts, nbins);
  SWZ_LAUNCH_CHECK(c);
  std::vector<uint32_t> starts(nbins + 1);
  SWZ_HIP(c, hipMemcpyAsync(starts.data(), d_starts, (nbins + 1) * 4, hipMemcpyDeviceToHost, c->stream));
  SWZ_HIP(c, hipStreamSynchronize(c->stream));
  *start_level = (int)estimate_start_level_host(starts, concurrency);
  return SWZ_OK;
}

int session_recon_ranks(swz_ctx* c, TileSession& t, int S, uint32_t child_bit, uint32_t* pos) {
  hipLaunchKernelGGL(recon_select_kernel, dim3(div_up(t.n, 256)), dim3(256), 0, c->stream, t.level, t.dup, t.n, S - 1, child_bit, pos);
  SWZ_LAUNCH_CHECK(c);
  SWZ_HIP(c, hipMemsetAsync(t.lb.counters, 0, CTR_COUNT * sizeof(uint32_t), c->stream));
  return scan_exclusive_u32(c, pos, pos, t.n, t.lb.counters + CTR_REMAINING, "rec");
}

int session_fast_reconstruct(swz_ctx* c, TileSession& t, const swz_tile_params& p, int S, int lowest_lv) {
  const uint32_t n = t.n;
  const double* bmin = t.bmin;
  const double* bmax = t.bmax;
  uint64_t* rkey = nullptr;
  uint32_t* ridx = nullptr;
  SWZ_TRY(c->get("recon_keys", (size_t)n, &rkey));
  SWZ_TRY(c->get("recon_idx", (size_t)n, &ridx));
  const uint32_t nb = div_up(n, 256);
  for (int lv = S - 1; lv >= lowest_lv; --lv) {
    const uint32_t child_bit = (lv + 1 == S) ? 0u : (1u << (lv + 1));
    SWZ_TRY(session_recon_ranks(c, t, S, child_bit, t.lb.flags));
    hipLaunchKernelGGL(recon_gather_kernel, dim3(nb), dim3(256), 0, c->stream, t.keys, n, t.lb.flags, t.level, t.dup,
                       S - 1, child_bit, rkey, ridx);
    SWZ_LAUNCH_CHECK(c);
    uint32_t m = 0;
    SWZ_TRY(read_u32(c, t.lb.counters + CTR_REMAINING, &m));
    if (m == 0) continue;
    LevelPlan plan = make_plan(lv - 1, p.sampler, p.max_points_per_node, p.spacing_at_root, p.max_depth, bmin,
                               bmax, true, false);
    plan.md_property = (p.flags & SWZ_FLAG_MIN_DISTANCE_PROPERTY) != 0;
    ActiveSet as{rkey, ridx, m};
    SWZ_TRY(session_need_positions(c, t, plan));
    LevelResult r;
    SWZ_TRY(level_step(c, plan, as, t.sp, t.lb, nullptr, nullptr, nullptr, &r));
    hipLaunchKernelGGL(recon_mark_kernel, dim3(div_up(m, 256)), dim3(256), 0, c->stream, ridx, m, t.lb.taken,
                       1u << lv, t.dup);
    SWZ_LAUNCH_CHECK(c);
    t.nodes += r.num_nodes;
    t.rounds += r.md_rounds;
  }
  return SWZ_OK;
}

int tile_device(swz_ctx* c, double* d_xyz, uint32_t n, const double bmin[3], const double bmax[3],
                const swz_tile_params& p, const TileDeviceOut& out_in, swz_tile_stats* stats) {
  TileDeviceOut out = out_in;
  if (p.strategy == SWZ_FAST && !out.dup) SWZ_TRY(c->get("fast_dup", (size_t)n, &out.dup));
  TileSession t;
  SWZ_TRY(session_prepare(c, t, d_xyz, n, bmin, bmax, p, out));
  if (p.strategy == SWZ_ACCURATE) {
    SWZ_TRY(session_run_levels(c, t, 20, -1, true));
    session_stats(t, stats);
    return SWZ_OK;
  }
  int S = 0;
  SWZ_TRY(fast_start_level(c, t.keys, n, p.fast_concurrency, &S));
  t.fast_start = S;
  t.next_level = S - 1;
  SWZ_TRY(session_run_levels(c, t, 20, -1));
  SWZ_TRY(session_fast_reconstruct(c, t, p, S, 0));
  session_stats(t, stats);
  return SWZ_OK;
}

__global__ __launch_bounds__(256) void count_taken_kernel(const uint8_t* __restrict__ taken, uint32_t n,
                                                          uint32_t* __restrict__ count) {
  const uint32_t i = blockIdx.x * 256 + threadIdx.x;
  const bool t = (i < n) && taken[i];
  const uint64_t b = __ballot(t);
  if (lane_id() == 0 && b) atomicAdd(count, (uint32_t)__popcll(b));
}

__global__ __launch_bounds__(256) void node_key_check_kernel(const uint64_t* __restrict__ keys, uint32_t n, uint32_t nsh,
                                                             uint64_t prefix, uint32_t* __restrict__ bad) {
  const uint32_t i = blockIdx.x * 256 + threadIdx.x;
  const bool b = i < n && (keys[i] >> nsh) != prefix;
  const uint64_t m = __ballot(b);
  if (lane_id() == 0 && m) atomicAdd(bad, (uint32_t)__popcll(m));
}

int sample_points_device(swz_ctx* c, int sampler, uint64_t max_points, const uint64_t* d_keys, const uint32_t* d_idx,
                         uint32_t n, const double* d_xyz, uint64_t node_key, int32_t node_level,
                         const double rmin[3], const double rmax[3], float spacing, int behaviour, uint8_t* d_taken,
                         uint64_t* num_taken) {
  const bool uses_node_key = greedy_sampler(sampler) || sampler == SWZ_JITTERED;
  if (node_level >= 0 && uses_node_key) {
    uint32_t* d_bad = nullptr;
    SWZ_TRY(c->get("lvl_counters", (size_t)CTR_COUNT, &d_bad));
    SWZ_HIP(c, hipMemsetAsync(d_bad, 0, sizeof(uint32_t), c->stream));
    const uint32_t nsh = level_shift(node_level);
    hipLaunchKernelGGL(node_key_check_kernel, dim3(div_up(n, 256)), dim3(256), 0, c->stream, d_keys, n, nsh,
                       node_key >> nsh, d_bad);
    SWZ_LAUNCH_CHECK(c);
    uint32_t bad = 0;
    SWZ_TRY(read_u32(c, d_bad, &bad));
    if (bad) return c->fail(SWZ_ERR_BAD_ARG, "swz_sample_points: " + std::to_string(bad) + " keys of the range do not lie in node_key's node");
  }
  double *X = nullptr, *Y = nullptr, *Z = nullptr;
  SWZ_TRY(c->get("sorted_x", (size_t)n, &X));
  SWZ_TRY(c->get("sorted_y", (size_t)n, &Y));
  SWZ_TRY(c->get("sorted_z", (size_t)n, &Z));
  SWZ_TRY(gather_positions(c, d_xyz, d_idx, n, X, Y, Z));
  LevelBuffers lb;
  SWZ_TRY(alloc_level_buffers(c, n, &lb));
  LevelPlan plan = make_plan(node_level, sampler, max_points, spacing, 100, rmin, rmax,
                             behaviour == SWZ_ALWAYS_ADHERE_TO_MIN_SPACING, false);
  if (!uses_node_key) plan.node_shift = 63;
  ActiveSet as{d_keys, nullptr, n};
  SortedPoints sp{X, Y, Z, d_xyz, d_idx};
  LevelResult r;
  SWZ_TRY(level_step(c, plan, as, sp, lb, nullptr, nullptr, nullptr, &r));
  SWZ_HIP(c, hipMemcpyAsync(d_taken, lb.taken, n, hipMemcpyDeviceToDevice, c->stream));
  if (num_taken) {
    SWZ_HIP(c, hipMemsetAsync(lb.counters, 0, sizeof(uint32_t), c->stream));
    hipLaunchKernelGGL(count_taken_kernel, dim3(div_up(n, 256)), dim3(256), 0, c->stream, lb.taken, n, lb.counters);
    SWZ_LAUNCH_CHECK(c);
    uint32_t cnt = 0;
    SWZ_TRY(read_u32(c, lb.counters, &cnt));
    *num_taken = cnt;
  }
  return SWZ_OK;
}

}
```

Before: 2692.

## Prebuild next MIN_DISTANCE level cell tables on a side stream during rounds

While the current chained MIN_DISTANCE level runs its sweep rounds, the next level's cell info and neighbour tables are built ahead of time on a low-priority build stream, using a double-buffered set of md_q buffers. When that level arrives it reuses the prebuilt tables and only launches the light state and start kernels. This hides table construction behind the rounds. It costs extra device memory for a second buffer set, adds cross-stream event synchronisation and buffer invalidation logic, and the side stream competes for compute with the main rounds.

```diff
diff --git a/schwarzwald_amd/csrc/swz_api.hip b/schwarzwald_amd/csrc/swz_api.hip
--- a/schwarzwald_amd/csrc/swz_api.hip
+++ b/schwarzwald_amd/csrc/swz_api.hip
@@ -87,6 +87,8 @@
 void swz_ctx::free_buf(swz::DevBuf& b) {
   if (b.ptr && b.ptr == sbi_clean_ptr) sbi_clean_ptr = nullptr;
   if (b.ptr && b.ptr == mq_qpos_buf) mq_qpos_buf = nullptr;
+  if (b.ptr && (b.ptr == mq_pre.cinfo || b.ptr == mq_pre.qnbr || b.ptr == mq_pre.rec || b.ptr == mq_pre.slot || b.ptr == mq_pre.qst))
+    mq_pre.valid = false;
   if (b.ptr) (void)(b.host ? hipHostFree(b.ptr) : hipFree(b.ptr));
   b.ptr = nullptr;
   b.cap = 0;
@@ -265,6 +267,7 @@
   c->prof_collect();
   for (hipEvent_t e : c->event_pool) (void)hipEventDestroy(e);
   for (hipStream_t st : c->aux_streams) (void)hipStreamDestroy(st);
+  if (c->mq_build_stream) (void)hipStreamDestroy(c->mq_build_stream);
   if (c->own_stream) (void)hipStreamDestroy(c->own_stream);
   delete c;
   return SWZ_OK;
diff --git a/schwarzwald_amd/csrc/swz_internal.h b/schwarzwald_amd/csrc/swz_internal.h
--- a/schwarzwald_amd/csrc/swz_internal.h
+++ b/schwarzwald_amd/csrc/swz_internal.h
@@ -33,6 +33,19 @@
   hipEvent_t e0, e1;
   uint64_t launches;
   uint64_t bytes;
+};
+
+struct MqPrebuild {
+  bool wanted = false;
+  uint32_t want_node_shift = 0, want_cl = 0, want_rg = 0;
+  bool valid = false;
+  uint32_t serial = 0;
+  int set = 0;
+  const void* akey = nullptr;
+  uint32_t m = 0, node_shift = 0, cl = 0, rg = 0, ncells = 0, nodes = 0;
+  const void *cinfo = nullptr, *qnbr = nullptr, *rec = nullptr, *slot = nullptr, *qst = nullptr;
+  hipEvent_t done = nullptr;
+  hipEvent_t t0 = nullptr, t1 = nullptr;
 };
 
 }
@@ -83,6 +96,11 @@
   const void* mq_qpos_buf = nullptr;
   const void* mq_qpos_keys = nullptr;
   uint32_t mq_qpos_m = 0;
+  hipStream_t mq_build_stream = nullptr;
+  swz::MqPrebuild mq_pre;
+  void prof_count(const char* name, uint64_t launches) {
+    if (profile) kstats[name].launches += launches;
+  }
   bool tiler_active = false;
   swz_tiler* nodes_tiler = nullptr;
   bool tiler_scratch_dead = false;
diff --git a/schwarzwald_amd/csrc/swz_md.h b/schwarzwald_amd/csrc/swz_md.h
--- a/schwarzwald_amd/csrc/swz_md.h
+++ b/schwarzwald_amd/csrc/swz_md.h
@@ -55,6 +55,8 @@
 
 int min_distance_keys_level(swz_ctx* c, const MdLevel& L, int cl, uint32_t* rounds_out, bool* used,
                             const MdShardRoot* shard_root = nullptr, bool* direct = nullptr);
+uint32_t key_sweep_record_granules(const swz_ctx* c, uint32_t cell_bits, double T);
+bool md_guess_chained_level(const swz_ctx* c, const LevelPlan& plan, const SortedPoints& sp, uint32_t points, MqPrebuild* want);
 int min_distance_block_level(swz_ctx* c, const MdLevel& L, bool* done);
 int min_distance_sparse_level(swz_ctx* c, const MdLevel& L, int cl, uint32_t* rounds_out, bool* used);
 int min_distance_rounds_level(swz_ctx* c, const MdLevel& L, uint32_t* rounds_out, bool* used);
diff --git a/schwarzwald_amd/csrc/swz_md.hip b/schwarzwald_amd/csrc/swz_md.hip
--- a/schwarzwald_amd/csrc/swz_md.hip
+++ b/schwarzwald_amd/csrc/swz_md.hip
@@ -181,6 +181,35 @@
   return cl;
 }
 
+bool md_guess_chained_level(const swz_ctx* c, const LevelPlan& plan, const SortedPoints& sp, uint32_t points, MqPrebuild* want) {
+  want->wanted = false;
+  if (plan.node_shift >= 63u || plan.node_shift < 3u || plan.node_shift % 3u != 0u || plan.terminal || plan.reroot || plan.md_property) return false;
+  const KeyMetric km = key_metric(c, plan, sp);
+  if (!km.ok) return false;
+  const uint32_t levels = (63u - plan.node_shift) / 3u;
+  if (levels > 6u) return false;
+  const double nodes = std::ldexp(1.0, 3 * (int)levels);
+  if (plan.force_sample ? points == 0u : (double)points / nodes <= (double)plan.max_points) return false;
+  auto occupied = [&](int cl) {
+    const double cells = nodes * std::ldexp(1.0, 3 * cl);
+    return std::max(1.0, cells * -std::expm1(-(double)points / cells));
+  };
+  const int cl_sparse = md_clamp_cell_levels((uint32_t)nodes, plan.cell_levels_geo);
+  if ((double)points / occupied(cl_sparse) < c->opt_num("SWZ_MD_SPARSE_LIMIT", 2.0)) return false;
+  int cl = plan.cell_levels_geo;
+  while (cl > 0 && plan.cell_levels_geo - cl < 3 && (double)points / occupied(cl) < 8.0) --cl;
+  cl = md_clamp_cell_levels((uint32_t)nodes, cl);
+  const double cells = nodes * std::ldexp(1.0, 3 * cl);
+  if (cells > 2147483632.0 || occupied(cl) / cells < c->opt_num("SWZ_MD_DIRECT_MIN_OCCUPANCY", 0.5)) return false;
+  const uint32_t cell_shift = plan.node_shift - 3u * (uint32_t)cl;
+  if (cell_shift / 3u > 21u) return false;
+  want->want_node_shift = plan.node_shift;
+  want->want_cl = (uint32_t)cl;
+  want->want_rg = key_sweep_record_granules(c, cell_shift / 3u, km.T);
+  want->wanted = true;
+  return true;
+}
+
 static int phases_cell_levels(swz_ctx* c, MdLevel& L, int* cl_out) {
   const LevelPlan& plan = L.plan;
   const double node_ext = (plan.root.maxx - plan.root.minx) / std::pow(2.0, plan.level + 1);
diff --git a/schwarzwald_amd/csrc/swz_mdkeys.h b/schwarzwald_amd/csrc/swz_mdkeys.h
--- a/schwarzwald_amd/csrc/swz_mdkeys.h
+++ b/schwarzwald_amd/csrc/swz_mdkeys.h
@@ -112,6 +112,8 @@
   uint32_t ncells = 0;
   uint32_t occ_cells = 0;
   uint32_t* d_cell_sums = nullptr;
+  int set = 0;
+  bool prebuilt = false;
   bool coded = false;
   bool lazy = false, big_cells = false;
   uint32_t groups = 1, ndense = 0;
@@ -126,6 +128,8 @@
 int mq_build_cell_tables(swz_ctx* c, MqLevel& q);
 int mq_list_dense_cells(swz_ctx* c, MqLevel& q);
 int mq_start_groups(swz_ctx* c, MqLevel& q);
+int mq_prebuild_launch(swz_ctx* c, MqLevel& q);
+int mq_prebuild_join(swz_ctx* c);
 uint32_t mq_sweep_grid(swz_ctx* c, const MqLevel& q);
 void mq_launch_round(const MqLevel& q, uint32_t g, uint32_t sweep_grid);
 void mq_set_round_word(hipStream_t stream, uint32_t* word, uint32_t value);
diff --git a/schwarzwald_amd/csrc/swz_mdkeys.hip b/schwarzwald_amd/csrc/swz_mdkeys.hip
--- a/schwarzwald_amd/csrc/swz_mdkeys.hip
+++ b/schwarzwald_amd/csrc/swz_mdkeys.hip
@@ -103,11 +103,15 @@
   return SWZ_OK;
 }
 
+uint32_t key_sweep_record_granules(const swz_ctx* c, uint32_t cell_bits, double T) {
+  const double r_cell = std::ldexp(1.0, (int)cell_bits) / T;
+  const uint32_t rg = (0.75 * r_cell * r_cell * r_cell <= 12.0) ? 4u : 8u;
+  return c->opt_int("SWZ_MD_KEYS_RG", rg) >= 8 ? 8u : 4u;
+}
+
 static int mq_choose_records_and_numbering(const swz_ctx* c, MqLevel& q, bool* direct_out) {
   MqArgs& a = q.a;
-  const double r_cell = std::ldexp(1.0, (int)a.cell_bits) / q.L.km.T;
-  a.rg = (0.75 * r_cell * r_cell * r_cell <= 12.0) ? 4u : 8u;
-  a.rg = c->opt_int("SWZ_MD_KEYS_RG", a.rg) >= 8 ? 8u : 4u;
+  a.rg = key_sweep_record_granules(c, a.cell_bits, q.L.km.T);
   a.rg2_shift = a.rg == 4u ? 3u : 4u;
   q.grid_entries = (uint64_t)q.L.sample_nodes * a.cells_per_node;
   const size_t per_cell = sizeof(uint2) + 32u * 4u + 2u * a.rg * sizeof(uint4) + 32u * 8u + sizeof(uint4) + 5u;
@@ -118,7 +122,9 @@
     size_t free_b = 0, total_b = 0, held = 0;
     if (hipMemGetInfo(&free_b, &total_b) != hipSuccess) free_b = 0;
     for (const auto& kv : c->bufs)
-      if (!kv.second.host && kv.first.compare(0, 4, "md_q") == 0) held += kv.second.cap;
+      if (!kv.second.host && kv.first.compare(0, 4, "md_q") == 0 &&
+          !(kv.first.size() > 2 && kv.first.compare(kv.first.size() - 2, 2, "_b") == 0))
+        held += kv.second.cap;
     max_cells = std::min<uint64_t>(max_cells, (uint64_t)((double)(free_b + held) * 0.9 / (double)per_cell));
   }
   const double occupancy = (double)q.L.occupied[q.cl] / (double)std::max<uint64_t>(1, q.grid_entries);
@@ -274,8 +280,18 @@
     }
   }
   if (fork) c->event_pool.push_back(fork);
-  return SWZ_OK;
-}
+  return mq_prebuild_join(c);
+}
+
+struct MqPrebuildGuard {
+  swz_ctx* c;
+  ~MqPrebuildGuard() {
+    if (c->mq_pre.done) {
+      (void)mq_prebuild_join(c);
+      c->mq_pre.valid = false;
+    }
+  }
+};
 
 struct MqTrace {
   bool on = false;
@@ -347,6 +363,8 @@
   mq_schedule(c, q);
   SWZ_TRY(mq_list_dense_cells(c, q));
   SWZ_TRY(mq_start_groups(c, q));
+  MqPrebuildGuard prebuild_guard{c};
+  SWZ_TRY(mq_prebuild_launch(c, q));
   MqTrace trace;
   mq_trace_begin(c, q, trace);
   SWZ_TRY(mq_run_rounds(c, q));
diff --git a/schwarzwald_amd/csrc/swz_mqbuild.hip b/schwarzwald_amd/csrc/swz_mqbuild.hip
--- a/schwarzwald_amd/csrc/swz_mqbuild.hip
+++ b/schwarzwald_amd/csrc/swz_mqbuild.hip
@@ -130,6 +130,56 @@
   uint32_t lazy;
 };
 
+__device__ __forceinline__ bool mq_adjacent_rel(const MqArgs& a, uint32_t rel, uint32_t k, uint32_t* nrel_out) {
+  const uint32_t all = (uint32_t)(a.cells_per_node - 1ull);
+  const uint32_t mz = all & 0x09249249u, my = mz << 1, mx = mz << 2;
+  const uint32_t v[3] = {rel & mx, rel & my, rel & mz};
+  const uint32_t mk[3] = {mx, my, mz};
+  const uint32_t d[3] = {k / 9u, (k / 3u) % 3u, k % 3u};
+  bool inside = true;
+  uint32_t nrel = 0;
+#pragma unroll
+  for (int ax = 0; ax < 3; ++ax) {
+    uint32_t w = v[ax];
+    if (d[ax] == 0u) {
+      inside &= w != 0u;
+      w = (w - 1u) & mk[ax];
+    } else if (d[ax] == 2u) {
+      inside &= w != mk[ax];
+      w = ((w | ~mk[ax]) + 1u) & mk[ax];
+    }
+    nrel |= w;
+  }
+  *nrel_out = nrel;
+  return inside;
+}
+
+__device__ __forceinline__ void mq_start_cell(const MqArgs& a, const MqStart& st, uint64_t cbase, uint32_t c, uint32_t k, bool in, uint32_t nb,
+                                              bool clear_qst) {
+  uint32_t best = 0;
+  if (st.lazy && in && k < 27u && nb != QNONE && (a.peers.shards <= 1u || (nb >> MQ_PEER_SHIFT) == 0u) && nb < c) best = nb + 1u;
+  if (st.lazy) {
+#pragma unroll
+    for (int off = 16; off >= 1; off >>= 1) best = max(best, (uint32_t)__shfl_xor((int)best, off, 32));
+    if (in && best && nb + 1u == best) {
+      const uint2 o = a.cinfo[best - 1u];
+      const uint32_t bq = o.x + (uint32_t)((float)(o.y - 1u - o.x) * a.lazy_frac);
+      a.slot[(size_t)(best - 1u) * 32 + (26u - k)] = (unsigned long long)bq;
+      a.qst[c] = make_uint4(a.cinfo[c].x, k, bq, 0u);
+    }
+  }
+  if (clear_qst && k == 2u && best == 0u) a.qst[c] = make_uint4(QNONE, 0u, 0u, 0u);
+  const bool push = in && k == 13u && best == 0u;
+  const uint32_t seg = (uint32_t)(cbase >> 3) & (a.nseg - 1u);
+  if (st.groups == 1u) {
+    mq_wave_push(push, c | MQ_WOKEN, st.queue[0] + (size_t)seg * a.segcap, st.qctr[0] + (size_t)seg * 32u);
+  } else {
+    const uint32_t g = push ? (a.direct ? c >> a.cpn_shift : a.csnode[c]) % st.groups : 0u;
+    for (uint32_t gg = 0; gg < st.groups; ++gg)
+      mq_wave_push(push && g == gg, c | MQ_WOKEN, st.queue[gg] + (size_t)seg * a.segcap, st.qctr[gg] + (size_t)seg * 32u);
+  }
+}
+
 __global__ __launch_bounds__(256) void mq_nbr_build_kernel(MqArgs a, uint32_t ncells, MqStart st) {
   for (uint64_t cbase = (uint64_t)blockIdx.x * 8u; cbase < ncells; cbase += (uint64_t)gridDim.x * 8u) {
     const uint32_t c = (uint32_t)cbase + threadIdx.x / 32u;
@@ -146,26 +196,8 @@
       nb = c;
     } else if (in && k < 27u) {
       const uint32_t rel = a.direct ? (c & (uint32_t)(a.cells_per_node - 1ull)) : a.crel[c];
-      const uint32_t all = (uint32_t)(a.cells_per_node - 1ull);
-      const uint32_t mz = all & 0x09249249u, my = mz << 1, mx = mz << 2;
-      const uint32_t v[3] = {rel & mx, rel & my, rel & mz};
-      const uint32_t mk[3] = {mx, my, mz};
-      const uint32_t d[3] = {k / 9u, (k / 3u) % 3u, k % 3u};
-      bool inside = true;
       uint32_t nrel = 0;
-#pragma unroll
-      for (int ax = 0; ax < 3; ++ax) {
-        uint32_t w = v[ax];
-        if (d[ax] == 0u) {
-          inside &= w != 0u;
-          w = (w - 1u) & mk[ax];
-        } else if (d[ax] == 2u) {
-          inside &= w != mk[ax];
-          w = ((w | ~mk[ax]) + 1u) & mk[ax];
-        }
-        nrel |= w;
-      }
-      if (inside) {
+      if (mq_adjacent_rel(a, rel, k, &nrel)) {
         if (a.peers.shards > 1u) {
           const uint32_t owner = (nrel >> (3u * (a.cell_levels - 1u))) * a.peers.shards / 8u;
           if (owner == a.peers.shard) {
@@ -184,28 +216,97 @@
       }
     }
     if (in) a.qnbr[(size_t)c * 32 + k] = nb;
-    uint32_t best = 0;
-    if (st.lazy && in && k < 27u && nb != QNONE && (a.peers.shards <= 1u || (nb >> MQ_PEER_SHIFT) == 0u) && nb < c) best = nb + 1u;
-    if (st.lazy) {
-#pragma unroll
-      for (int off = 16; off >= 1; off >>= 1) best = max(best, (uint32_t)__shfl_xor((int)best, off, 32));
-      if (in && best && nb + 1u == best) {
-        const uint2 o = a.cinfo[best - 1u];
-        const uint32_t bq = o.x + (uint32_t)((float)(o.y - 1u - o.x) * a.lazy_frac);
-        a.slot[(size_t)(best - 1u) * 32 + (26u - k)] = (unsigned long long)bq;
-        a.qst[c] = make_uint4(a.cinfo[c].x, k, bq, 0u);
+    mq_start_cell(a, st, cbase, c, k, in, nb, a.direct && in_grid);
+  }
+}
+
+__global__ __launch_bounds__(256) void mq_cinfo_early_kernel(const uint64_t* __restrict__ akey, uint32_t m, uint32_t cell_shift, uint32_t ncells,
+                                                             uint2* __restrict__ cinfo, uint32_t vec) {
+  const uint64_t i0 = ((uint64_t)blockIdx.x * 256u + threadIdx.x) * 4u;
+  if (i0 >= m) return;
+  const uint32_t n = m - i0 < 4u ? (uint32_t)(m - i0) : 4u;
+  uint64_t key[6];
+  if (vec && n == 4u) {
+    const ulonglong2 v0 = *reinterpret_cast<const ulonglong2*>(akey + i0), v1 = *reinterpret_cast<const ulonglong2*>(akey + i0 + 2);
+    key[1] = v0.x, key[2] = v0.y, key[3] = v1.x, key[4] = v1.y;
+  } else {
+#pragma unroll
+    for (uint32_t j = 0; j < 4u; ++j) key[1 + j] = j < n ? akey[i0 + j] : 0ull;
+  }
+  key[0] = i0 ? akey[i0 - 1u] : 0ull;
+  key[5] = i0 + 4u < m ? akey[i0 + 4u] : 0ull;
+#pragma unroll
+  for (uint32_t j = 0; j < 4u; ++j) {
+    if (j >= n) break;
+    const uint32_t i = (uint32_t)i0 + j;
+    const uint64_t pre = key[1 + j] >> cell_shift;
+    const bool first = i == 0u || (key[j] >> cell_shift) != pre;
+    const bool last = i + 1u == m || (key[2 + j] >> cell_shift) != pre;
+    if ((!first && !last) || pre >= ncells) continue;
+    if (first) cinfo[pre].x = i;
+    if (last) cinfo[pre].y = i + 1u;
+  }
+}
+
+__global__ __launch_bounds__(256) void mq_nbr_early_kernel(MqArgs a, uint32_t ncells) {
+  for (uint64_t cbase = (uint64_t)blockIdx.x * 8u; cbase < ncells; cbase += (uint64_t)gridDim.x * 8u) {
+    const uint32_t c = (uint32_t)cbase + threadIdx.x / 32u;
+    const uint32_t k = threadIdx.x & 31u;
+    if (c >= ncells) continue;
+    const uint2 ci = a.cinfo[c];
+    if (k < 2u) a.rec[((size_t)c << a.rg2_shift) + k * a.rg] = make_uint4(ci.x, 0u, k, ci.y);
+    if (k == 2u) a.qst[c] = make_uint4(QNONE, 0u, 0u, 0u);
+    if (ci.x == ci.y) continue;
+    uint32_t nb = QNONE;
+    if (k == 13u) {
+      nb = c;
+    } else if (k < 27u) {
+      const uint32_t rel = c & (uint32_t)(a.cells_per_node - 1ull);
+      uint32_t nrel = 0;
+      if (mq_adjacent_rel(a, rel, k, &nrel)) {
+        const uint32_t g = (c - rel) | nrel;
+        const uint2 cn = a.cinfo[g];
+        if (cn.x != cn.y) nb = g;
       }
     }
-    if (a.direct && in_grid && k == 2u && best == 0u) a.qst[c] = make_uint4(QNONE, 0u, 0u, 0u);
-    const bool push = in && k == 13u && best == 0u;
-    const uint32_t seg = (uint32_t)(cbase >> 3) & (a.nseg - 1u);
-    if (st.groups == 1u) {
-      mq_wave_push(push, c | MQ_WOKEN, st.queue[0] + (size_t)seg * a.segcap, st.qctr[0] + (size_t)seg * 32u);
-    } else {
-      const uint32_t g = push ? (a.direct ? c >> a.cpn_shift : a.csnode[c]) % st.groups : 0u;
-      for (uint32_t gg = 0; gg < st.groups; ++gg)
-        mq_wave_push(push && g == gg, c | MQ_WOKEN, st.queue[gg] + (size_t)seg * a.segcap, st.qctr[gg] + (size_t)seg * 32u);
-    }
+    a.qnbr[(size_t)c * 32 + k] = nb;
+  }
+}
+
+__global__ __launch_bounds__(256) void mq_state_late_kernel(const uint8_t* __restrict__ gone, uint32_t m, uint8_t* __restrict__ state, uint32_t vec) {
+  const uint64_t i0 = ((uint64_t)blockIdx.x * 256u + threadIdx.x) * 16u;
+  if (i0 >= m) return;
+  if (vec && m - i0 >= 16u) {
+    const uint4 g = *reinterpret_cast<const uint4*>(gone + i0);
+    const uint32_t w[4] = {g.x, g.y, g.z, g.w};
+    uint32_t s[4];
+#pragma unroll
+    for (int q = 0; q < 4; ++q) {
+      uint32_t sw = 0x01010101u * (uint32_t)QS_OPEN;
+#pragma unroll
+      for (int j = 0; j < 4; ++j)
+        if ((w[q] >> (8 * j)) & 0xFFu) sw = (sw & ~(0xFFu << (8 * j))) | ((uint32_t)QS_DEAD << (8 * j));
+      s[q] = sw;
+    }
+    *reinterpret_cast<uint4*>(state + i0) = make_uint4(s[0], s[1], s[2], s[3]);
+  } else {
+    for (uint64_t i = i0; i < m && i < i0 + 16u; ++i) state[i] = gone[i] ? (uint8_t)QS_DEAD : (uint8_t)QS_OPEN;
+  }
+}
+
+__global__ __launch_bounds__(256) void mq_start_late_kernel(MqArgs a, uint32_t ncells, MqStart st) {
+  for (uint64_t cbase = (uint64_t)blockIdx.x * 8u; cbase < ncells; cbase += (uint64_t)gridDim.x * 8u) {
+    const uint32_t c = (uint32_t)cbase + threadIdx.x / 32u;
+    const uint32_t k = threadIdx.x & 31u;
+    bool in = c < ncells;
+    if (in) {
+      const uint2 ci = a.cinfo[c];
+      in = ci.x != ci.y;
+    }
+    uint32_t nb = QNONE;
+    if (in && k == 13u) nb = c;
+    else if (in && k < 27u && st.lazy) nb = a.qnbr[(size_t)c * 32 + k];
+    mq_start_cell(a, st, cbase, c, k, in, nb, false);
   }
 }
 
@@ -237,6 +338,16 @@
   }
   q.occ_cells = a.direct ? std::max(1u, std::min<uint32_t>(q.L.occupied[q.cl], q.ncells)) : q.ncells;
   return SWZ_OK;
+}
+
+static bool mq_prebuilt_matches(const swz_ctx* c, const MqLevel& q) {
+  const MqPrebuild& p = c->mq_pre;
+  const MqArgs& a = q.a;
+  const MdLevel& L = q.L;
+  return p.valid && !p.done && c->opt_on("SWZ_MD_PREBUILD", true) && !q.sharded && p.akey == (const void*)a.akey && p.m == a.m &&
+         p.node_shift == L.plan.node_shift && p.cl == (uint32_t)q.cl && p.rg == a.rg && a.direct != 0u &&
+         a.cells_per_node == (1ull << (3u * p.cl)) && L.sample_nodes == p.nodes && a.all_sampled != 0u && L.num_nodes == p.nodes &&
+         p.nodes == (1ull << (63u - L.plan.node_shift)) && p.ncells == q.ncells && a.gone != nullptr && a.keep_qpos != 0u;
 }
 
 int mq_alloc_arrays(swz_ctx* c, MqLevel& q) {
@@ -254,25 +365,39 @@
   c->mq_qpos_keys = as.akey;
   c->mq_qpos_m = m;
   SWZ_TRY(c->get(("md_qovf" + sfx).c_str(), (size_t)m, &a.ovf));
-  SWZ_TRY(c->get(("md_qcinfo" + sfx).c_str(), (size_t)ncells, &a.cinfo));
+  MqPrebuild& pre = c->mq_pre;
+  q.prebuilt = mq_prebuilt_matches(c, q);
+  q.set = q.prebuilt ? pre.set : 0;
+  const std::string cs = sfx + (q.set ? "_b" : "");
+  SWZ_TRY(c->get(("md_qcinfo" + cs).c_str(), (size_t)ncells, &a.cinfo));
   if (!a.direct) {
     uint32_t* cellbuf = nullptr;
     SWZ_TRY(c->get(("md_qcells" + sfx).c_str(), (size_t)ncells * 2, &cellbuf));
     a.crel = cellbuf;
     a.csnode = cellbuf + ncells;
   }
-  SWZ_TRY(c->get(("md_qnbr" + sfx).c_str(), (size_t)ncells * 32, &a.qnbr));
-  SWZ_TRY(c->get(("md_qrec" + sfx).c_str(), (size_t)ncells * 2 * a.rg, &a.rec));
-  SWZ_TRY(c->get(("md_qslot" + sfx).c_str(), (size_t)ncells * 32, &a.slot));
-  SWZ_TRY(c->get(("md_qst" + sfx).c_str(), (size_t)ncells, &a.qst));
-  SWZ_HIP(c, memset_large(a.slot, 0xFF, (size_t)ncells * 32 * sizeof(unsigned long long), c->stream));
+  SWZ_TRY(c->get(("md_qnbr" + cs).c_str(), (size_t)ncells * 32, &a.qnbr));
+  SWZ_TRY(c->get(("md_qrec" + cs).c_str(), (size_t)ncells * 2 * a.rg, &a.rec));
+  SWZ_TRY(c->get(("md_qslot" + cs).c_str(), (size_t)ncells * 32, &a.slot));
+  SWZ_TRY(c->get(("md_qst" + cs).c_str(), (size_t)ncells, &a.qst));
+  if (q.prebuilt && !(pre.valid && pre.cinfo == a.cinfo && pre.qnbr == a.qnbr && pre.rec == a.rec && pre.slot == a.slot && pre.qst == a.qst))
+    q.prebuilt = false;
+  if (pre.valid) c->prof_count(q.prebuilt ? "mq_prebuild_taken" : "mq_prebuild_dropped", 1);
+  pre.valid = false;
+  if (!q.prebuilt) SWZ_HIP(c, memset_large(a.slot, 0xFF, (size_t)ncells * 32 * sizeof(unsigned long long), c->stream));
   return SWZ_OK;
 }
 
 int mq_build_cell_tables(swz_ctx* c, MqLevel& q) {
   MqArgs& a = q.a;
   const uint32_t m = a.m, ncells = q.ncells;
-  if (a.direct) {
+  if (q.prebuilt) {
+    hipLaunchKernelGGL(mq_state_late_kernel, dim3(div_up(m, 4096)), dim3(256), 0, c->stream, a.gone, m, a.state,
+                       (((uintptr_t)a.gone | (uintptr_t)a.state) & 15u) == 0 ? 1u : 0u);
+    SWZ_LAUNCH_CHECK(c);
+    c->prof_count("mq_tables_late", 1);
+  } else if (a.direct) {
+    c->prof_count("mq_tables_at_setup", 1);
     SWZ_HIP(c, memset_large(a.cinfo, 0, (size_t)ncells * sizeof(uint2), c->stream));
     hipLaunchKernelGGL(mq_direct_build_kernel, dim3(div_up(m, 1024)), dim3(256), 0, c->stream, a,
                        ((uintptr_t)a.akey & 15u) == 0 ? 1u : 0u);
@@ -353,10 +478,177 @@
     start.queue[g] = ag.queue[0];
     start.qctr[g] = ag.qctr;
   }
-  hipLaunchKernelGGL(mq_nbr_build_kernel, dim3(std::min<uint32_t>(div_up(ncells, 8), 1u << 20)), dim3(256), 0, c->stream, q.ga[0], ncells, start);
+  const dim3 nbr_grid(std::min<uint32_t>(div_up(ncells, 8), 1u << 20));
+  if (q.prebuilt) {
+    hipLaunchKernelGGL(mq_start_late_kernel, nbr_grid, dim3(256), 0, c->stream, q.ga[0], ncells, start);
+    c->prof_count("mq_tables_late", 1);
+  } else {
+    hipLaunchKernelGGL(mq_nbr_build_kernel, nbr_grid, dim3(256), 0, c->stream, q.ga[0], ncells, start);
+    if (a.direct) c->prof_count("mq_tables_at_setup", 1);
+  }
   SWZ_LAUNCH_CHECK(c);
   SWZ_STAGE(c, "mq tables");
   return SWZ_OK;
 }
 
-}
+int mq_prebuild_launch(swz_ctx* c, MqLevel& q) {
+  MqPrebuild& p = c->mq_pre;
+  if (!p.wanted) return SWZ_OK;
+  p.wanted = false;
+  p.valid = false;
+  const MqArgs& a = q.a;
+  if (!a.direct || q.sharded || q.groups + 1u > 4u || p.want_node_shift >= 63u) return SWZ_OK;
+  const uint32_t rg = p.want_rg, cl = p.want_cl;
+  const uint64_t nodes = 1ull << (63u - p.want_node_shift);
+  const uint64_t ncells = nodes << (3u * cl);
+  if (ncells > 0x7FFFFFF0ull) return SWZ_OK;
+  const std::string cs = q.set ? "" : "_b";
+  const char* base[5] = {"md_qcinfo", "md_qnbr", "md_qrec", "md_qslot", "md_qst"};
+  const size_t bytes[5] = {ncells * sizeof(uint2), ncells * 32 * 4, ncells * 2 * rg * sizeof(uint4), ncells * 32 * 8, ncells * sizeof(uint4)};
+  if (const char* mc = c->opt("SWZ_MD_DIRECT_MAX_CELLS")) {
+    if ((uint64_t)q.ncells + ncells > (uint64_t)std::max(0LL, atoll(mc))) return SWZ_OK;
+  }
+  size_t grow = 0;
+  bool grows[5] = {false, false, false, false, false};
+  for (int i = 0; i < 5; ++i) {
+    const auto it = c->bufs.find(base[i] + cs);
+    grows[i] = it == c->bufs.end() || it->second.cap < bytes[i];
+    if (grows[i]) grow += bytes[i] + bytes[i] / 16 + 256;
+  }
+  if (grow) {
+    size_t free_b = 0, total_b = 0;
+    if (hipMemGetInfo(&free_b, &total_b) != hipSuccess) free_b = 0;
+    if ((double)grow > (double)free_b * 0.9) return SWZ_OK;
+  }
+  uint2* cinfo = nullptr;
+  uint32_t* qnbr = nullptr;
+  uint4* rec = nullptr;
+  unsigned long long* slot = nullptr;
+  uint4* qst = nullptr;
+  void* got[5] = {nullptr, nullptr, nullptr, nullptr, nullptr};
+  for (int i = 0; i < 5; ++i)
+    if (c->get((base[i] + cs).c_str(), bytes[i], &got[i]) != SWZ_OK) {
+      c->err.clear();
+      (void)hipGetLastError();
+      for (int j = 0; j < 5; ++j) {
+        const auto it = c->bufs.find(base[j] + cs);
+        if (grows[j] && it != c->bufs.end()) c->free_buf(it->second);
+      }
+      return SWZ_OK;
+    }
+  cinfo = static_cast<uint2*>(got[0]);
+  qnbr = static_cast<uint32_t*>(got[1]);
+  rec = static_cast<uint4*>(got[2]);
+  slot = static_cast<unsigned long long*>(got[3]);
+  qst = static_cast<uint4*>(got[4]);
+  MqArgs e{};
+  e.akey = a.akey;
+  e.m = a.m;
+  e.direct = 1u;
+  e.cpn_shift = 3u * cl;
+  e.cells_per_node = 1ull << (3u * cl);
+  e.cell_shift = p.want_node_shift - 3u * cl;
+  e.rg = rg;
+  e.rg2_shift = rg == 4u ? 3u : 4u;
+  e.cinfo = cinfo;
+  e.qnbr = qnbr;
+  e.rec = rec;
+  e.qst = qst;
+  e.peers.shards = 1u;
+  hipError_t bad = hipSuccess;
+  auto ok = [&](hipError_t r) {
+    if (bad == hipSuccess && r != hipSuccess) bad = r;
+    return bad == hipSuccess;
+  };
+  if (!c->mq_build_stream) {
+    int least = 0, greatest = 0;
+    if (ok(hipDeviceGetStreamPriorityRange(&least, &greatest)) && !ok(hipStreamCreateWithPriority(&c->mq_build_stream, hipStreamNonBlocking, least)))
+      c->mq_build_stream = nullptr;
+  }
+  hipStream_t bs = c->mq_build_stream;
+  hipEvent_t fork = c->take_event();
+  p.done = c->take_event();
+  const bool timed = c->opt("SWZ_DEBUG") != nullptr;
+  if (timed) {
+    p.t0 = c->take_event();
+    p.t1 = c->take_event();
+  }
+  if (bs && fork && p.done && (!timed || (p.t0 && p.t1)) && ok(hipEventRecord(fork, c->stream)) && ok(hipStreamWaitEvent(bs, fork, 0))) {
+    if (timed) ok(hipEventRecord(p.t0, bs));
+    if (ok(memset_large(cinfo, 0, bytes[0], bs))) {
+      hipLaunchKernelGGL(mq_cinfo_early_kernel, dim3(div_up(e.m, 1024)), dim3(256), 0, bs, e.akey, e.m, e.cell_shift, (uint32_t)ncells, cinfo,
+                         ((uintptr_t)e.akey & 15u) == 0 ? 1u : 0u);
+      ok(hipGetLastError());
+    }
+    if (ok(memset_large(slot, 0xFF, bytes[3], bs))) {
+      hipLaunchKernelGGL(mq_nbr_early_kernel, dim3(std::min<uint32_t>(div_up(ncells, 8), 1u << 20)), dim3(256), 0, bs, e, (uint32_t)ncells);
+      ok(hipGetLastError());
+    }
+    if (timed) ok(hipEventRecord(p.t1, bs));
+    ok(hipEventRecord(p.done, bs));
+  } else if (bad == hipSuccess) {
+    bad = hipErrorUnknown;
+  }
+  if (fork) c->event_pool.push_back(fork);
+  if (bad != hipSuccess) {
+    (void)hipGetLastError();
+    if (bs) (void)hipStreamSynchronize(bs);
+    for (hipEvent_t* ev : {&p.done, &p.t0, &p.t1}) {
+      if (*ev) c->event_pool.push_back(*ev);
+      *ev = nullptr;
+    }
+    return SWZ_OK;
+  }
+  if (c->opt("SWZ_TRACE")) {
+    const hipError_t te = hipStreamSynchronize(bs);
+    fprintf(stderr, "[swz trace] %s:%d %s -> %s\n", __FILE__, __LINE__, "mq tables ahead", hipGetErrorString(te));
+    fflush(stderr);
+  }
+  c->prof_count("mq_tables_ahead", 2);
+  p.set = q.set ? 0 : 1;
+  p.akey = a.akey;
+  p.m = a.m;
+  p.node_shift = p.want_node_shift;
+  p.cl = cl;
+  p.rg = rg;
+  p.ncells = (uint32_t)ncells;
+  p.nodes = (uint32_t)nodes;
+  p.cinfo = cinfo;
+  p.qnbr = qnbr;
+  p.rec = rec;
+  p.slot = slot;
+  p.qst = qst;
+  p.valid = true;
+  ++p.serial;
+  return SWZ_OK;
+}
+
+int mq_prebuild_join(swz_ctx* c) {
+  MqPrebuild& p = c->mq_pre;
+  if (!p.done) return SWZ_OK;
+  hipError_t e = hipStreamWaitEvent(c->stream, p.done, 0);
+  if (e != hipSuccess) {
+    (void)hipGetLastError();
+    p.valid = false;
+    e = c->mq_build_stream ? hipStreamSynchronize(c->mq_build_stream) : hipSuccess;
+  }
+  c->event_pool.push_back(p.done);
+  p.done = nullptr;
+  if (p.t0 && p.t1) {
+    float ms = 0.f;
+    (void)hipEventSynchronize(p.t1);
+    (void)hipEventElapsedTime(&ms, p.t0, p.t1);
+    fprintf(stderr, "[swz] MIN_DISTANCE tables built ahead: %u cells (cell levels %u, records of %u), %.2f ms on the build stream\n", p.ncells, p.cl,
+            p.rg - 1u, ms);
+    c->event_pool.push_back(p.t0);
+    c->event_pool.push_back(p.t1);
+  }
+  p.t0 = p.t1 = nullptr;
+  if (e != hipSuccess) {
+    (void)hipGetLastError();
+    p.valid = false;
+  }
+  return SWZ_OK;
+}
+
+}
diff --git a/schwarzwald_amd/csrc/swz_session.hip b/schwarzwald_amd/csrc/swz_session.hip
--- a/schwarzwald_amd/csrc/swz_session.hip
+++ b/schwarzwald_amd/csrc/swz_session.hip
@@ -75,6 +75,8 @@
   const bool chain_static = chains && first_mode < 0 && t.params.sampler == SWZ_MIN_DISTANCE &&
                             !(t.params.flags & SWZ_FLAG_MIN_DISTANCE_PROPERTY) && !t.sp.ghosts && !t.front && !c->shard &&
                             !c->md_shard_root && c->opt_on("SWZ_MD_DEFER", true);
+  const bool prebuild = chain_static && c->opt_on("SWZ_MD_PREBUILD", true);
+  c->mq_pre.valid = false;
   LevelChain chain;
   chain.max_gone = c->opt_num("SWZ_MD_DEFER_MAX_GONE", 0.125);
   for (int level = t.next_level; (t.as.gone ? t.as.live : t.as.m) > 0 && level <= last_level; ++level) {
@@ -87,10 +89,12 @@
                                t.params.max_depth, t.bmin, t.bmax, false, true);
     plan.md_property = (t.params.flags & SWZ_FLAG_MIN_DISTANCE_PROPERTY) != 0;
     chain.may_defer = false;
+    c->mq_pre.wanted = false;
     if (chain_static && level < 20) {
       const LevelPlan next = make_plan(level + 1, t.params.sampler, t.params.max_points_per_node, t.params.spacing_at_root,
                                        t.params.max_depth, t.bmin, t.bmax, false, true);
       chain.may_defer = !plan.terminal && !plan.reroot && !next.terminal && !next.reroot;
+      if (chain.may_defer && prebuild) (void)md_guess_chained_level(c, next, t.sp, t.as.gone ? t.as.live : t.as.m, &c->mq_pre);
     }
     if (chain.may_defer || t.as.gone) plan.take_code = (uint8_t)(level + 2);
     if (first_mode >= 0 && level == t.next_level) plan.md_property = false;
@@ -105,7 +109,14 @@
     LevelResult r;
     t.as.parent_prefix = pprefix;
     t.as.parents = pprefix ? parents : 0u;
-    SWZ_TRY(level_step(c, plan, t.as, t.sp, t.lb, t.level, t.key_buf[t.which], t.idx_buf[t.which], &r, &chain));
+    const uint32_t found_tables = c->mq_pre.valid ? c->mq_pre.serial : 0u;
+    const int step_status = level_step(c, plan, t.as, t.sp, t.lb, t.level, t.key_buf[t.which], t.idx_buf[t.which], &r, &chain);
+    c->mq_pre.wanted = false;
+    SWZ_TRY(step_status);
+    if (found_tables && c->mq_pre.valid && c->mq_pre.serial == found_tables && !r.needs_flush) {
+      c->mq_pre.valid = false;
+      c->prof_count("mq_prebuild_dropped", 1);
+    }
     if (r.needs_flush) {
       if (!t.as.gone) return c->fail(SWZ_ERR_INTERNAL, "a level outside a chain asked for the chain's compaction");
       uint32_t remaining = 0;
```

New measurement: 2723, median of 6. 1.1% higher.
